# wwood/CoverM

Hardware: AMD Instinct MI355X
Metric: aligned reads/s through coverm contig (mean trimmed_mean covered_fraction variance) (higher is better)
Workload: dtype i32 depth / u64 sums / f32 estimators

## Files before the change

coverm_amd/csrc/covermhip.hip:

```cpp
#include "pileup_kernels.hip.h"
#include "prep_lean.hip.h"
#include "genome_kernels.hip.h"
#include "sep_kernels.hip.h"
#include "ingest_kernels.hip.h"
#include "group_kernels.hip.h"
#include "sam_kernels.hip.h"

#include <algorithm>
#include <atomic>
#include <cstddef>
#include <chrono>
#include <cstdio>
#include <dlfcn.h>
#include <functional>
#include <sched.h>
#include <cstdlib>
#include <cstring>
#include <map>
#include <mutex>
#include <string>
#include <future>
#include <thread>
#include <vector>

#include "../../include/covermhip.h"
#include "roctx_ranges.h"
#include "knobs.h"
#include "record_store.h"
#include "store_plan_core.h"

using namespace covk;

static_assert(sizeof(cov_config) == 40 && offsetof(cov_config, min_aligned_length) == 12 && offsetof(cov_config, min_percent_identity) == 16 &&
              offsetof(cov_config, contig_end_exclusion) == 24 && offsetof(cov_config, want) == 32, "cov_config layout");
static_assert(sizeof(cov_batch) == 80 && offsetof(cov_batch, cigar) == 64 && offsetof(cov_batch, n_records) == 72, "cov_batch layout");
static_assert(sizeof(cov_contig_stats) == 128 && offsetof(cov_contig_stats, sum_identity_primary) == 40 && offsetof(cov_contig_stats, win_sum_d) == 56 &&
              offsetof(cov_contig_stats, first_record) == 88 && offsetof(cov_contig_stats, win_min_d) == 104 && offsetof(cov_contig_stats, hist_len) == 112 &&
              offsetof(cov_contig_stats, hist_off) == 120, "cov_contig_stats layout");
static_assert(sizeof(cov_summary) == 32 && offsetof(cov_summary, hist_total) == 24, "cov_summary layout");
static_assert(sizeof(cov_interval) == 24 && sizeof(cov_interval_stats) == 56, "interval struct layout");
static_assert(sizeof(cov_genome_stats) == 24 && sizeof(cov_genome_stats) == sizeof(covk::DevGenomeStats) && offsetof(cov_genome_stats, genome_len) == offsetof(covk::DevGenomeStats, genome_len) &&
              offsetof(cov_genome_stats, any_nonzero) == offsetof(covk::DevGenomeStats, any_nonzero), "cov_genome_stats mirrors the device struct");
static_assert(sizeof(cov_genome_entry) == 24 && offsetof(cov_genome_entry, first_tid) == 8 && offsetof(cov_genome_entry, gid) == 12 && offsetof(cov_genome_entry, n_contigs_seen) == 16 &&
              offsetof(cov_genome_entry, any_nonzero) == 20 && sizeof(covk::SepEntry) == 8, "cov_genome_entry layout (numpy mirror in coverm_amd/native.py)");
static_assert(sizeof(cov_estimator) == sizeof(covk::DevEstimator) && offsetof(cov_estimator, contig_end_exclusion) == offsetof(covk::DevEstimator, excl) &&
              offsetof(cov_estimator, trim_max) == offsetof(covk::DevEstimator, trim_max) && COV_EST_MAX == covk::EST_MAX && COV_EST_ANIR == covk::EST_ANIR, "cov_estimator mirrors the device struct");

namespace {

#define HIPCHK(call)                                                                          \
    do {                                                                                      \
        hipError_t e_ = (call);                                                               \
        if (e_ != hipSuccess) {                                                               \
            char b_[512];                                                                     \
            snprintf(b_, sizeof b_, "%s failed: %s (%s:%d)", #call, hipGetErrorString(e_), __FILE__, __LINE__); \
            s->err = b_;                                                                      \
            return COV_ERR_HIP;                                                               \
        }                                                                                     \
    } while (0)

std::string g_create_error;

// ... 131 lines not shown
    uint64_t ing_first_record = 0;
    uint64_t ing_launched = 0;
    covi::BgzfBlock *h_blocks = nullptr; size_t h_blocks_cap = 0;
    uint64_t ing_comp = 0, ing_infl = 0, ing_blocks = 0;
    bool ing_active = false;
    InflateKernel ing_K;
    hipStream_t ing_copy = nullptr;
    std::future<hipError_t> ing_prep;
    hipEvent_t ing_ev[COV_INGEST_SLOTS] = {}, ing_fed = nullptr;
    double ing_s_alloc = 0;
    double ing_s_part[4] = {0, 0, 0, 0};

    bool sam_active = false, sam_seen_record = false, sam_decode_timed = false;
    uint64_t sam_window = 0, sam_expected = 0, sam_lines = 0, sam_bytes = 0, sam_err_line = 0;
    uint32_t sam_err = 0, sam_k = 0;
    DevBuf<uint8_t> m_text[2], m_blob;
    DevBuf<u64> m_nl, m_tab, m_res, m_noff;
    DevBuf<u32> m_line_end, m_cnt, m_rec_idx, m_cig_idx, m_bsum[3], m_slots;
    samc::Table m_names{};
    hipEvent_t sam_buf_free[2] = {}, sam_ev[4] = {};
    float sam_ms = 0.f; uint32_t sam_launches = 0;

    bool finished = false;
    uint8_t *h_res = nullptr; size_t h_res_cap = 0;
    std::future<std::pair<uint8_t *, size_t>> h_res_prep;
    DevContig *h_ctg = nullptr;
    DevGlobal h_glob{};
    bool last_gen_all = false;
    uint64_t algo_bytes = 0;

    hipEvent_t ev[COV_K_COUNT][2] = {};
    hipEvent_t ev_begin[COV_K_COUNT] = {};
    int ev_fresh = -1;
    float k_ms[COV_K_COUNT] = {};
    uint32_t k_launches[COV_K_COUNT] = {};
};

static cov_status spill_store(cov_session *s, bool &progress);

namespace {

size_t result_block_bytes(u32 n_targets) { return sizeof(DevGlobal) + (size_t)std::max<u32>(n_targets, 1) * sizeof(DevContig); }
static size_t result_host_bytes(const cov_session *s, u32 nT) {
    return result_block_bytes(nT) + (size_t)std::max<u32>(nT, 1) * ((s->have_mask || s->have_runs) ? 1u : std::max<u32>(s->est.n, 1u)) * sizeof(float);
}
static void result_host_take(cov_session *s) {
    if (!s->h_res_prep.valid()) return;
    const std::pair<uint8_t *, size_t> r = s->h_res_prep.get();
    if (!r.first) return;
    if (r.second > s->h_res_cap) {
        if (s->h_res) (void)hipHostFree(s->h_res);
        s->h_res = r.first; s->h_res_cap = r.second;
    } else (void)hipHostFree(r.first);
}

hipError_t bind_result_block(cov_session *s, u32 n_targets) {
    hipError_t e = s->d_res.reserve(result_block_bytes(n_targets) + (size_t)std::max<u32>(n_targets, 1) * COV_EST_MAX * sizeof(float), s->stream);
    if (e != hipSuccess) return e;
    s->d_glob.p = reinterpret_cast<DevGlobal *>(s->d_res.p); s->d_glob.cap = 1;
    s->d_ctg.p = reinterpret_cast<DevContig *>(s->d_res.p + sizeof(DevGlobal)); s->d_ctg.cap = std::max<u32>(n_targets, 1);
    return hipSuccess;
}

Records records_of(const cov_session *s) {
    Records r{};
    if (s->adopted) {
// ... 36 lines not shown
        const cov_status sp = spill_store(s, progress);
        if (sp != COV_OK) return sp;
        s->spill_retry_at = progress ? 0 : 2 * s->store.n_records;
    }
    if (s->store.n_records + n >= 0xfffffff0ull) { s->err = "more than 2^32 records of one reference (or of one batch) in the record store"; return COV_ERR_INVALID_ARG; }
    if (s->store.n_cigar + ncig >= 0xfffffff0ull) { s->err = "more than 2^32 CIGAR words of one reference (or of one batch) in the record store"; return COV_ERR_INVALID_ARG; }
    RecordStore &S = s->store;
    const uint64_t R = S.n_records, N = R + n; hipStream_t st = s->stream;
    HIPCHK(S.reserve(N, S.n_cigar + ncig + 1, st, R, S.n_cigar, false));
    HIPCHK(S.copy_in(*b, n, off0, ncig, kind, st));
    if (off0 != (u32)S.n_cigar) {
        const u32 cnt = (u32)(n + 1);
        hipLaunchKernelGGL(k_rebase_offsets, dim3((cnt + 255) / 256), dim3(256), 0, st, S.cigar_off.p + R, cnt, off0, (u32)S.n_cigar);
        HIPCHK(hipGetLastError());
    }
    S.n_records = N; S.n_cigar += ncig;
    s->finished = false;
    if (!from_device) HIPCHK(hipStreamSynchronize(st));
    return COV_OK;
}

cov_status materialise_adopted(cov_session *s) {
    if (!s->adopted) return COV_OK;
    const cov_batch ab = s->adopted_batch;
    s->adopted = false; s->store.n_records = 0; s->store.n_cigar = 0;
    return append(s, &ab, true);
}

void timing_events(cov_session *s) {
    if (s->ev[0][0]) return;
    for (int k = 0; k < COV_K_COUNT; k++)
        for (int j = 0; j < 2; j++) (void)hipEventCreate(&s->ev[k][j]);
}
void time_begin(cov_session *s, int k) {
    if (s->ev_fresh >= 0) { s->ev_begin[k] = s->ev[s->ev_fresh][1]; return; }
    (void)hipEventRecord(s->ev[k][0], s->stream); s->ev_begin[k] = s->ev[k][0];
}
void time_end(cov_session *s, int k) { (void)hipEventRecord(s->ev[k][1], s->stream); s->k_launches[k]++; s->ev_fresh = k; }

template <bool H, int TABLES>
void launch_fast_v(cov_session *s, const PileupArgs &a, u32 n_tiles) {
    const auto kern = TABLES == 1 ? &k_pileup_fast<H> : &k_pileup_fast2t<H>;
    const size_t smem = pileup_fast_smem_bytes(H, TABLES == 1 ? FAST_HB : FAST_HB7, TABLES);
    static std::atomic<int> occ_dev[64];
    std::atomic<int> &occ_slot = occ_dev[(unsigned)s->cfg.device & 63u];
    int occ = occ_slot.load(std::memory_order_relaxed);
    const u32 chunk = (u32)s->chunk_tiles;
    const u32 n_chunks = (n_tiles + chunk - 1) / chunk;
    if (!occ) {
        (void)hipFuncSetAttribute(reinterpret_cast<const void *>(kern), hipFuncAttributeMaxDynamicSharedMemorySize, (int)smem);
        int nb = 0;
        if (hipOccupancyMaxActiveBlocksPerMultiprocessor(&nb, reinterpret_cast<const void *>(kern), 256, smem) != hipSuccess || nb < 1) {
            (void)hipGetLastError();
            nb = (int)std::max<size_t>(1, std::min<size_t>(8, (160 * 1024) / smem));
        }
        occ = nb; occ_slot.store(nb, std::memory_order_relaxed);
    }
    const u32 wg_per_cu = 8u * (u32)occ;
    const u32 grid = std::max(1u, std::min((n_chunks + 3) / 4, (u32)s->n_cus * wg_per_cu));
    hipLaunchKernelGGL(kern, dim3(grid), dim3(256), smem, s->stream, a, n_tiles, chunk);
}
template <bool H>
void launch_fast_t(cov_session *s, const PileupArgs &a, u32 n_tiles) {
    if (s->fast_tables == 2) launch_fast_v<H, 2>(s, a, n_tiles);
    else launch_fast_v<H, 1>(s, a, n_tiles);
}

template <bool H, bool W>
void launch_stream_t(cov_session *s, const PileupArgs &a, u32 n_tiles, bool slow_list_only = false) {
    const size_t smem = pileup_stream_smem_bytes();
    static std::atomic<int> occ_dev[64];
    std::atomic<int> &occ_slot = occ_dev[(unsigned)s->cfg.device & 63u];
    int occ = occ_slot.load(std::memory_order_relaxed);
    const u32 chunk = (u32)s->chunk_tiles;
    const u32 n_chunks = (n_tiles + chunk - 1) / chunk;
    if (!occ) {
        (void)hipFuncSetAttribute(reinterpret_cast<const void *>(&k_pileup_stream<H, W>), hipFuncAttributeMaxDynamicSharedMemorySize, (int)smem);
        int nb = 0;
        if (hipOccupancyMaxActiveBlocksPerMultiprocessor(&nb, reinterpret_cast<const void *>(&k_pileup_stream<H, W>), 256, smem) != hipSuccess || nb < 1) {
            (void)hipGetLastError();
            nb = (int)std::max<size_t>(1, std::min<size_t>(8, (160 * 1024) / smem));
        }
        occ = nb; occ_slot.store(nb, std::memory_order_relaxed);
    }
    const u32 wg_per_cu = 8u * (u32)occ;
    if (slow_list_only) {
        hipLaunchKernelGGL((k_pileup_stream<H, W>), dim3((u32)s->n_cus), dim3(256), smem, s->stream, a, 0u, 1u,
                           (const u32 *)s->d_slow_list.p, (const u32 *)&s->d_glob.p->n_slow);
        return;
    }
    const u32 grid = std::max(1u, std::min((n_chunks + 3) / 4, (u32)s->n_cus * wg_per_cu));
    hipLaunchKernelGGL((k_pileup_stream<H, W>), dim3(grid), dim3(256), smem, s->stream, a, n_tiles, chunk, (const u32 *)nullptr,
                       (const u32 *)nullptr);
}
template <bool H, bool W>
void launch_any_pileup(cov_session *s, const PileupArgs &a, u32 n_tiles) {
    if (s->use_fast && !W) {
        launch_fast_t<H>(s, a, n_tiles);
        launch_stream_t<H, W>(s, a, n_tiles, true);
    } else launch_stream_t<H, W>(s, a, n_tiles);
}

PileupArgs pileup_args(cov_session *s) {
    PileupArgs a{};
    a.tile_contig = s->d_tile_contig.p; a.tile_start = s->d_tile_start.p; a.desc = s->d_desc.p;
    a.runs = s->d_runs.p; a.cx_runs = s->d_cx_runs.p; a.r = records_of(s); a.ctg = s->d_ctg.p; a.g = s->d_glob.p;
    a.hist_arena = s->d_arena.p; a.excl = s->cfg.contig_end_exclusion; a.depth_out = nullptr; a.tile_base = 0;
    return a;
}

}

extern "C" {

int cov_abi_version(void) { return COVERMHIP_ABI_VERSION; }

const char *cov_last_error(const cov_session *s) { return s ? s->err.c_str() : g_create_error.c_str(); }

static hipError_t ingest_prepare_(cov_session *s) {
    hipError_t e = hipSetDevice(s->cfg.device);
    if (e != hipSuccess || s->ing_copy) return e;
#define PREP(x) do { e = (x); if (e != hipSuccess) return e; } while (0)
    PREP(hipStreamCreateWithFlags(&s->ing_copy, hipStreamNonBlocking));
    for (int k = 0; k < COV_INGEST_SLOTS; k++) PREP(hipEventCreateWithFlags(&s->ing_ev[k], hipEventDisableTiming));
    PREP(hipEventCreateWithFlags(&s->ing_fed, hipEventDisableTiming));
    PREP(hipStreamCreateWithFlags(&s->ing_aux, hipStreamNonBlocking));
    PREP(hipStreamCreateWithFlags(&s->ing_parse, hipStreamNonBlocking));
    s->ing_ext = s->ing_parse;
    for (int k = 0; k < 2; k++) { PREP(hipEventCreateWithFlags(&s->ing_inf_done[k], hipEventDisableTiming)); PREP(hipEventCreateWithFlags(&s->ing_lz_done[k], hipEventDisableTiming)); }
    for (int k = 0; k < 4; k++) PREP(hipEventCreateWithFlags(&s->ing_ver_done[k], hipEventDisableTiming));
    for (int k = 0; k < 3; k++) { PREP(hipEventCreateWithFlags(&s->ing_ext_done[k], hipEventDisableTiming)); PREP(hipEventCreateWithFlags(&s->ing_cdone[k], hipEventDisableTiming)); }
// ... 20 lines not shown
    const bool timing = cov_timing_on();
    const auto tc0 = std::chrono::steady_clock::now();
    auto stamp = [&](const char *what) { if (timing) fprintf(stderr, "[covermhip] cov_create: %s at %.4fs\n", what, std::chrono::duration<double>(std::chrono::steady_clock::now() - tc0).count()); };
    int ndev = 0;
    hipError_t e = hipGetDeviceCount(&ndev);
    stamp("hipGetDeviceCount (runtime initialised)");
    if (e != hipSuccess || ndev <= 0) {
        g_create_error = std::string("no usable HIP device: ") + hipGetErrorString(e) +
                         " (the engine has no CPU fallback)";
        return COV_ERR_HIP;
    }
    if (cfg->device < 0 || cfg->device >= ndev) { g_create_error = "device ordinal out of range"; return COV_ERR_INVALID_ARG; }
    e = hipSetDevice(cfg->device);
    if (e != hipSuccess) { g_create_error = std::string("hipSetDevice: ") + hipGetErrorString(e); return COV_ERR_HIP; }
    cov_session *s = new cov_session();
    s->cfg = *cfg;
    {
        const char *mode = getenv("COVERM_PILEUP");
        if (mode && !strcmp(mode, "stream")) s->use_fast = false;
        s->tile = STREAM_TW;
        stamp("hipSetDevice");
        int cus = 0;
        if (hipDeviceGetAttribute(&cus, hipDeviceAttributeMultiprocessorCount, cfg->device) == hipSuccess && cus > 0) s->n_cus = cus;
        stamp("device attribute");
    }
    if (cfg->want & COV_WANT_INGEST) s->ing_prep = std::async(std::launch::async, [s] { return ingest_prepare_(s); });
    if (const char *el = getenv("COVERM_EST_LANES")) s->est_lanes = atoi(el) ? 1 : 0;
    if (const char *ft = getenv("COVERM_FAST_TABLES")) s->fast_tables = atoi(ft) == 2 ? 2 : 1;
    if (const char *pk = getenv("COVERM_PREP_KERNEL")) s->prep_kernel = atoi(pk) == 7 ? 7 : 0;
    if (const char *im = getenv("COVERM_IDENTITY")) s->id_mode = strcmp(im, "serial") ? 1 : 0;
    { long long v; if (covknob::get("store_cap_records", v) && v >= 1) s->cap_records = std::min<uint64_t>((uint64_t)v, 0xfffffff0ull); }
    { long long v; if (covknob::get("store_cap_cigar", v) && v >= 1) s->cap_cigar = std::min<uint64_t>((uint64_t)v, 0xfffffff0ull); }
    { long long v; if (covknob::get("pileup_chunk_tiles", v) && v >= 1 && v <= 64) s->chunk_tiles = (int)v; }
    e = hipEventCreateWithFlags(&s->ev_prep_done, hipEventDisableTiming);
    if (e == hipSuccess) e = hipEventCreateWithFlags(&s->ev_side_done, hipEventDisableTiming);
    if (e == hipSuccess) e = hipStreamCreateWithFlags(&s->stream, hipStreamNonBlocking);
    if (e != hipSuccess) { g_create_error = std::string("hipStreamCreate: ") + hipGetErrorString(e); (void)ingest_prep_wait(s); delete s; return COV_ERR_HIP; }
    stamp("streams and events");
    e = bind_result_block(s, 1);
    if (e != hipSuccess) { g_create_error = std::string("hipMalloc: ") + hipGetErrorString(e); cov_destroy(s); return COV_ERR_HIP; }
    stamp("first hipMalloc");
    *out = s;
    return COV_OK;
}

static void ingest_free_buffers(cov_session *s) {
    s->g_scratch.release(); s->g_carry.release(); s->g_blocks.release(); s->g_status.release();
    s->g_crc_tab.release();
    for (int k = 0; k < 3; k++) { s->g_win[k].release(); s->g_cwin[k].release(); }
    for (int k = 0; k < 4; k++) { s->g_seg[k].release(); s->g_recbase[k].release(); s->g_cigbase[k].release(); }
    s->g_tok.release(); s->g_ntok.release(); s->g_tok2.release(); s->g_ntok2.release();
    for (auto &b : s->m_text) b.release();
    s->m_nl.release(); s->m_tab.release(); s->m_line_end.release(); s->m_cnt.release(); s->m_rec_idx.release(); s->m_cig_idx.release();
}

void cov_destroy(cov_session *s) {
    if (!s) return;
    (void)ingest_prep_wait(s);
    (void)hipSetDevice(s->cfg.device);
    if (s->stream) (void)hipStreamSynchronize(s->stream);
    s->d_tlen.release(); s->d_tile_contig.release(); s->d_tile_start.release(); s->d_mask.release();
    s->d_grow.release(); s->d_gtids.release(); s->d_gseg_genome.release(); s->d_gseg_start.release(); s->d_genomes.release(); s->d_ghist.release(); s->d_ghist_top.release(); s->d_order.release();
    s->d_sgid.release(); s->d_sblk.release(); s->d_sent_pos.release(); s->d_stop_last1.release(); s->d_stop_first.release(); s->d_scounts.release(); s->d_scode.release();
    s->d_stop_cnt.release(); s->d_stop_seg.release(); s->d_sent.release();
    s->d_gout.release(); if (s->h_gout) (void)hipHostFree(s->h_gout); s->h_gout = nullptr;
    s->d_tile_first.release(); s->d_tcnt.release(); s->d_fov.release(); s->d_tscan.release(); s->d_ttop.release(); s->d_slow_list.release();
    s->d_ctg_scratch.release(); s->d_depth_all.release(); s->d_depth_off.release(); s->d_iv.release(); s->d_ivst.release(); s->d_ivhist.release();
    s->d_cx_list.release(); s->d_cx_cnt.release(); s->d_cx_cur.release(); s->d_cx_scan.release(); s->d_cx_top.release(); s->d_cx_runs.release();
    if (s->side) {
        (void)hipStreamSynchronize(s->side);
        if (s->side_owned) (void)hipStreamDestroy(s->side);
        s->side = nullptr; s->side_owned = false;
    }
    if (s->ing_aux) (void)hipStreamSynchronize(s->ing_aux);
    if (s->ing_parse) (void)hipStreamSynchronize(s->ing_parse);
    if (s->ing_ext) (void)hipStreamSynchronize(s->ing_ext);
    ingest_free_buffers(s);
    s->g_result.release();
    if (s->ing_aux) (void)hipStreamDestroy(s->ing_aux);
    if (s->ing_parse) (void)hipStreamDestroy(s->ing_parse);
    for (int k = 0; k < 2; k++) { if (s->ing_inf_done[k]) (void)hipEventDestroy(s->ing_inf_done[k]); if (s->ing_lz_done[k]) (void)hipEventDestroy(s->ing_lz_done[k]); }
    for (int k = 0; k < 4; k++) if (s->ing_ver_done[k]) (void)hipEventDestroy(s->ing_ver_done[k]);
    for (int k = 0; k < 3; k++) { if (s->ing_ext_done[k]) (void)hipEventDestroy(s->ing_ext_done[k]); if (s->ing_cdone[k]) (void)hipEventDestroy(s->ing_cdone[k]); }
    if (s->h_winres) (void)hipHostFree(s->h_winres);
    s->h_winres = nullptr;
    if (s->h_blocks) (void)hipHostFree(s->h_blocks);
    s->h_blocks = nullptr;
    if (s->ing_copy) { (void)hipStreamSynchronize(s->ing_copy); (void)hipStreamDestroy(s->ing_copy); }
    for (int k = 0; k < COV_INGEST_SLOTS; k++) if (s->ing_ev[k]) (void)hipEventDestroy(s->ing_ev[k]);
    for (hipEvent_t e : s->sam_buf_free) if (e) (void)hipEventDestroy(e);
    for (hipEvent_t e : s->sam_ev) if (e) (void)hipEventDestroy(e);
    for (auto &b : s->m_text) b.release();
    s->m_blob.release(); s->m_nl.release(); s->m_tab.release(); s->m_res.release(); s->m_noff.release(); s->m_line_end.release(); s->m_cnt.release();
    s->m_rec_idx.release(); s->m_cig_idx.release(); s->m_slots.release(); for (auto &b : s->m_bsum) b.release();
    if (s->ing_fed) (void)hipEventDestroy(s->ing_fed);
    s->d_res.release(); s->d_ctg.p = nullptr; s->d_glob.p = nullptr; s->d_desc.release(); s->d_gather.release();
    if (s->h_gather) (void)hipHostFree(s->h_gather);
    s->h_gather = nullptr;
    result_host_take(s);
    if (s->h_res) (void)hipHostFree(s->h_res);
    s->h_res = nullptr; s->h_res_cap = 0; s->h_ctg = nullptr;
    if (s->h_chist) (void)hipHostFree(s->h_chist);
    s->h_chist = nullptr; s->h_chist_cap = 0;
    s->h_estf = nullptr; s->store.release();
    s->d_runs.release(); s->d_part.release(); s->d_prep_args.release(); s->d_gen_list.release(); s->d_hist_top.release(); s->d_ident.release(); s->d_identp.release(); s->d_idch.release();
    if (s->ev_prep_done) (void)hipEventDestroy(s->ev_prep_done);
    if (s->ev_side_done) (void)hipEventDestroy(s->ev_side_done); s->d_arena.release(); s->d_chist.release(); s->d_depth.release();
    for (int k = 0; k < COV_K_COUNT; k++)
        for (int j = 0; j < 2; j++) if (s->ev[k][j]) (void)hipEventDestroy(s->ev[k][j]);
    if (s->stream) (void)hipStreamDestroy(s->stream);
    delete s;
}

static void genomes_off(cov_session *s) {
    if (s->have_genomes && (s->cfg.want & COV_WANT_IDENTITY_NONSUPP_ONLY))
        for (uint32_t k = 0; k < s->est.n; k++)
            if (s->est.e[k].kind == COV_EST_ANIR) { s->est = EstParams{}; s->est_valid = false; break; }
    s->have_genomes = false; s->have_runs = false; s->gen_valid = false;
}
cov_status cov_set_targets(cov_session *s, uint32_t n_targets, const uint64_t *target_len) {
    if (!s || (!target_len && n_targets)) return COV_ERR_INVALID_ARG;
    HIPCHK(hipSetDevice(s->cfg.device));
    s->n_targets = n_targets;
    s->h_tlen.resize(n_targets);
    s->h_tile_first.assign((size_t)n_targets + 1, 0);
    uint64_t nt = 0;
    for (uint32_t c = 0; c < n_targets; c++) {
        if (target_len[c] > 0x7fffffffull) { s->err = "target length exceeds BAM's i32 range"; return COV_ERR_INVALID_ARG; }
        s->h_tlen[c] = (uint32_t)target_len[c];
        s->h_tile_first[c] = (uint32_t)nt;
        nt += (target_len[c] + (uint64_t)s->tile - 1) / (uint64_t)s->tile;
    }
    if (nt >= 0x7fffffffull) { s->err = "too many tiles"; return COV_ERR_INVALID_ARG; }
    s->h_tile_first[n_targets] = (uint32_t)nt;
    s->n_tiles = (uint32_t)nt;
    std::vector<u32> tc(nt), ts(nt);
    for (uint32_t c = 0; c < n_targets; c++) {
        u32 k = s->h_tile_first[c];
        for (uint64_t p = 0; p < target_len[c]; p += (uint64_t)s->tile, k++) { tc[k] = c; ts[k] = (u32)p; }
    }
    HIPCHK(s->d_tlen.reserve(std::max<size_t>(1, n_targets), s->stream));
    HIPCHK(s->d_tile_contig.reserve(std::max<size_t>(1, nt), s->stream));
// ... 165 lines not shown
        return COV_OK;
    }
    { const cov_status st = materialise_adopted(s); if (st) return st; }
    return append(s, b, true);
}

cov_status cov_ingest_abort(cov_session *s) {
    if (!s) return COV_ERR_INVALID_ARG;
    if (!s->ing_active) return COV_OK;
    HIPCHK(hipSetDevice(s->cfg.device));
    s->ing_active = false; s->sam_active = false;
    for (hipStream_t st : {s->ing_copy, s->stream, s->ing_aux, s->ing_parse, s->ing_ext})
        if (st) HIPCHK(hipStreamSynchronize(st));
    s->ing_rec_total = s->ing_cig_total = 0; s->ing_round_n = 0; s->ing_fail = 0;
    s->ing_extracted = s->ing_batch;
    if (s->ing_rec_spilled) {
        s->ing_rec_spilled = 0;
        s->err = "cov_ingest_abort: part of the file had already left the bounded record store; cov_reset the session";
        return COV_ERR_STATE;
    }
    return COV_OK;
}

cov_status cov_reset(cov_session *s) {
    if (!s) return COV_ERR_INVALID_ARG;
    if (s->ing_active) {
        const bool spilled = s->ing_rec_spilled != 0;
        const cov_status a = cov_ingest_abort(s);
        if (a != COV_OK && !(spilled && a == COV_ERR_STATE)) return a;
        if (a != COV_OK) s->err.clear();
    }
    s->adopted = false; s->store.n_records = 0; s->store.n_cigar = 0; s->finished = false; s->depth_all_valid = false; s->store.mates_valid = 0; s->ing_was_span = false;
    s->spill.clear(); s->merged_valid = false; s->merged_hist.clear(); s->ing_rec_spilled = 0; s->spill_retry_at = 0; s->spill_est.clear(); s->est_valid = false; s->gen_valid = false;
    return COV_OK;
}

static cov_status convert_results(cov_session *s, const DevGlobal &G, const DevContig *ctg, uint64_t n_records, cov_contig_stats *stats,
                                  cov_summary *summary, int64_t min_ok_tid = -1, uint64_t rec_base = 0) {
    const u32 nT = s->n_targets;
    const bool want_hist = s->cfg.want & COV_WANT_HIST;
    if (G.internal_error) { s->err = "internal error: depth or histogram size exceeded its proven bound"; return COV_ERR_STATE; }
    uint64_t err_rec = ~0ull; int err_code = 0;
    if (G.first_error != ~0ull) { err_rec = G.first_error >> 8; err_code = (int)(G.first_error & 0xff); }
    const u32 n_chunks = nT >= 65536u ? std::min<u32>(8u, std::max<u32>(1u, std::thread::hardware_concurrency())) : 1u;
    const u32 per_chunk = (nT + n_chunks - 1) / std::max<u32>(n_chunks, 1u);
    auto chunked = [&](auto fn) {
        if (n_chunks <= 1) { fn(0u, 0u, nT); return; }
        std::vector<std::thread> th;
        for (u32 k = 1; k < n_chunks; k++) th.emplace_back([&, k] { fn(k, std::min(nT, k * per_chunk), std::min(nT, (k + 1) * per_chunk)); });
        fn(0u, 0u, std::min(nT, per_chunk));
        for (auto &t : th) t.join();
    };
    const bool want_hist_bins = want_hist;
    const u64 excl = s->cfg.contig_end_exclusion;
    std::vector<uint64_t> ch_last(n_chunks, 0), ch_bins(n_chunks, 0), ch_unsorted(n_chunks, ~0ull);
    std::vector<uint8_t> ch_any(n_chunks, 0);
    if (n_chunks > 1)
        chunked([&](u32 k, u32 lo, u32 hi) {
            uint64_t last = 0, bins = 0; bool any = false;
            for (u32 c = lo; c < hi; c++) {
                const DevContig &C = ctg[c];
                if (C.n_pass == 0) continue;
                last = any ? std::max<uint64_t>(last, C.last_rec) : C.last_rec; any = true;
                if (want_hist_bins) {
                    const u64 L = s->h_tlen[c];
                    if (2 * excl < L && (!s->have_mask || s->h_mask[c])) bins += C.max_d + 1u;
// ... 76 lines not shown
static cov_status verdict_results(cov_session *s, const DevGlobal &G, uint64_t unsorted_at, uint64_t n_records, cov_summary *summary) {
    if (G.internal_error) { s->err = "internal error: depth or histogram size exceeded its proven bound"; return COV_ERR_STATE; }
    uint64_t err_rec = ~0ull; int err_code = 0;
    if (G.first_error != ~0ull) { err_rec = G.first_error >> 8; err_code = (int)(G.first_error & 0xff); }
    if (unsorted_at != ~0ull && unsorted_at <= err_rec) {
        s->err = "BAM file appears to be unsorted. Input BAM files must be sorted by reference (i.e. by samtools sort)";
        return COV_ERR_UNSORTED;
    }
    if (err_code) {
        char b[256];
        const char *what = err_code == 2 ? "Mapping record encountered that does not have an 'NM' auxiliary tag in the SAM/BAM format"
                         : err_code == 3 ? "Unexpected data type of NM aux tag"
                         : err_code == 4 ? "aligned block starts at or beyond the end of its reference sequence"
                         : err_code == 7 ? "record refers to a reference id outside the header (Corrupt BAM file?)"
                                         : "invalid CIGAR operation";
        snprintf(b, sizeof b, "%s (record %llu)", what, (unsigned long long)err_rec);
        s->err = b;
        return (cov_status)err_code;
    }
    if (summary) {
        uint64_t prim = 0, cons = 0;
        for (u32 k = 0; k < COUNTER_SLOTS * 8; k++) { prim += G.prim_slots[k]; cons += G.cons_slots[k]; }
        summary->num_detected_primary_alignments = prim; summary->n_records = n_records; summary->n_considered = cons; summary->hist_total = 0;
    }
    return COV_OK;
}

static cov_status finish_once(cov_session *s, cov_contig_stats *stats, cov_summary *summary, bool &again);

static cov_status finish_store(cov_session *s, cov_contig_stats *stats, cov_summary *summary) {
    bool again = false;
    cov_status st = finish_once(s, stats, summary, again);
    if (st == COV_OK && again) st = finish_once(s, stats, summary, again);
    if (st == COV_OK && again) { s->err = "internal error: bucket sizing did not converge"; return COV_ERR_STATE; }
    return st;
}

static cov_status merge_spilled(cov_session *s, cov_contig_stats *stats, cov_summary *summary);

cov_status cov_finish(cov_session *s, cov_contig_stats *stats, cov_summary *summary) {
    covr::Range rr("cov_finish");
    if (s) s->merged_valid = false;
    cov_summary local;
    cov_status st = finish_store(s, stats, (s && s->spill.active && !summary) ? &local : summary);
    if (st == COV_OK && s->spill.active) st = merge_spilled(s, stats, summary ? summary : &local);
    return st;
}

cov_status cov_finish_genomes(cov_session *s, cov_summary *summary) {
    covr::Range rr("cov_finish_genomes");
    if (!s) return COV_ERR_INVALID_ARG;
    s->merged_valid = false;
    if (s->spill.active) { s->err = "cov_finish_genomes: part of the sample's contigs left the bounded record store: cov_finish, and aggregate on the host"; return COV_ERR_STATE; }
    s->lean_finish = true;
    const cov_status st = finish_store(s, nullptr, summary);
    s->lean_finish = false;
    return st;
}

static cov_status finish_once(cov_session *s, cov_contig_stats *stats, cov_summary *summary, bool &again) {
    again = false;
    if (!s || (!stats && s->n_targets && !s->lean_finish)) return COV_ERR_INVALID_ARG;
    const bool lean = s->lean_finish;
    s->depth_all_valid = false;
    HIPCHK(hipSetDevice(s->cfg.device));
    timing_events(s);
// ... 12 lines not shown
    const uint64_t ncig_all = s->adopted ? s->adopted_ncig : s->store.n_cigar;
    const bool long_cigars = R && ncig_all / R >= 16;
    const int prep_kernel = s->prep_kernel;
    const int prep_passes = long_cigars ? 1 : 2 * PREP_PASSES, prep_b = 1;
    const u32 prep_chunk = (u32)(256 * prep_b * prep_passes);
    const u32 prep_grid = (R + prep_chunk - 1) / prep_chunk;
    HIPCHK(s->d_part.reserve((size_t)prep_grid + 2, st));
    if (want_id) {
        if (!(s->cfg.want & COV_WANT_IDENTITY_PRIMARY_ONLY)) HIPCHK(s->d_ident.reserve(std::max<size_t>(1, R), st));
        if (!(s->cfg.want & COV_WANT_IDENTITY_NONSUPP_ONLY)) HIPCHK(s->d_identp.reserve(std::max<size_t>(1, R), st));
        HIPCHK(s->d_idch.reserve((size_t)R / ID_CH + 2, st));
    }
    if (want_hist) HIPCHK(s->d_arena.reserve((size_t)R + nT + 1, st));

    TileIdx ti{};
    ti.tile_first = s->d_tile_first.p; ti.tcnt = s->d_tcnt.p; ti.fov = s->d_fov.p; ti.shift = s->tile_shift; ti.n_tiles = s->n_tiles;
    CxIdx cx{};
    {
        const uint64_t ncig_now = s->adopted ? s->adopted_ncig : s->store.n_cigar;
        HIPCHK(s->d_cx_list.reserve((size_t)(ncig_now / CX_MIN_OPS) + 64, st));
        cx.list = s->d_cx_list.p; cx.list_cap = (u32)std::min<uint64_t>(ncig_now / CX_MIN_OPS + 64, 0xffffffffull);
        cx.cnt = s->d_cx_cnt.p; cx.cur = s->d_cx_cur.p; cx.cscan = s->d_cx_scan.p; cx.ctop = s->d_cx_top.p;
        cx.runs = s->d_cx_runs.p; cx.runs_cap = s->d_cx_runs.cap;
    }
    const Records r = records_of(s);
    const uint8_t *mask = s->have_mask ? s->d_mask.p : nullptr;
    FilterCfg f{};
    f.include_improper_pairs = s->cfg.include_improper_pairs; f.include_supplementary = s->cfg.include_supplementary;
    f.include_secondary = s->cfg.include_secondary; f.filter_single = s->cfg.filter_single;
    f.min_mapq = s->cfg.min_mapq; f.min_aligned_length = s->cfg.min_aligned_length;
    f.min_percent_identity = s->cfg.min_percent_identity; f.min_aligned_percent = s->cfg.min_aligned_percent;
    double *idp = (want_id && !(s->cfg.want & COV_WANT_IDENTITY_NONSUPP_ONLY)) ? s->d_identp.p : nullptr;
    double *idn = (want_id && !(s->cfg.want & COV_WANT_IDENTITY_PRIMARY_ONLY)) ? s->d_ident.p : nullptr;
    HIPCHK(s->d_prep_args.reserve(1, st));
    HIPCHK(s->d_gen_list.reserve((size_t)R / 64 + 2, st));
    PrepArgs pa{};
    {
        PrepHot &ph = pa.hot;
        ph.tid = r.tid; ph.pos = r.pos; ph.flag = r.flag; ph.nmk = r.nm_kind; ph.nm = r.nm; ph.coff = r.cigar_off; ph.cigar = r.cigar; ph.mapq = r.mapq; ph.lseq = r.l_seq;
        ph.runs = s->d_runs.p; ph.tcnt = ti.tcnt; ph.fov = ti.fov; ph.identp = idp; ph.identn = idn;
        ph.n = r.n; ph.cigar_end = r.cigar_end; ph.n_targets = nT; ph.shift = ti.shift; ph.steps = (u32)prep_chunk / 256u;
        ph.gate_mask = 0x4u | (f.include_secondary ? 0u : 0x100u) | (f.include_supplementary ? 0u : 0x800u) | (f.include_improper_pairs ? 0u : 0x2u);
        ph.p1_mask = 0x4u | (f.include_secondary ? 0u : 0x100u) | (f.include_supplementary ? 0u : 0x800u);
        ph.min_mapq = f.min_mapq; ph.min_aligned_length = f.min_aligned_length; ph.min_percent_identity = f.min_percent_identity; ph.min_aligned_percent = f.min_aligned_percent;
        PrepCold &pc = pa.cold;
        pc.ctg = s->d_ctg.p; pc.g = s->d_glob.p; pc.part = s->d_part.p; pc.cx_list = cx.list; pc.mask = mask; pc.tlen = s->d_tlen.p; pc.tile_first = s->d_tile_first.p;
        pc.cx_list_cap = cx.list_cap; pc.gen_list = s->d_gen_list.p;
    }
    hipLaunchKernelGGL(k_init, dim3((std::max(std::max(nT, COUNTER_SLOTS * 8), s->n_tiles) + 255) / 256), dim3(256), 0, st, s->d_ctg.p,
                       nT, s->d_glob.p, ti, cx, s->d_prep_args.p, pa);
    HIPCHK(hipGetLastError());

    if (R) {
        time_begin(s, COV_K_PREP);
        const u32 n_steps = (R + 63u) / 64u;
        const bool gen_all = prep_kernel != 7 && (uint64_t)R < (uint64_t)nT * 128u;
        s->last_gen_all = gen_all;
        const u32 gen_grid = gen_all ? std::min<u32>((u32)s->n_cus * 64u, (n_steps + 3u) / 4u) : std::min<u32>((u32)s->n_cus * 8u, (n_steps + 3u) / 4u);
#define COV_LAUNCH_PREP(ID, FI, MA)                                                                                                       \
        do {                                                                                                                              \
            if (prep_kernel == 7)                                                                                                         \
                hipLaunchKernelGGL((k_prep7s<ID, FI, MA>), dim3(prep_grid), dim3(256), 0, st, r, s->d_tlen.p, nT, mask, f, s->d_ctg.p,   \
                                   s->d_glob.p, s->d_runs.p, idp, idn, s->d_part.p, ti, prep_passes, prep_b, cx.list, cx.list_cap);      \
            else if (gen_all)                                                                                                             \
                hipLaunchKernelGGL((k_prep_generic<ID, FI, MA>), dim3(gen_grid), dim3(256), 0, st, (const PrepArgs *)s->d_prep_args.p, n_steps); \
            else {                                                                                                                        \
                hipLaunchKernelGGL((k_prep_lean<ID, FI, MA>), dim3(prep_grid), dim3(256), 0, st, pa.hot, (const PrepArgs *)s->d_prep_args.p); \
                hipLaunchKernelGGL((k_prep_generic<ID, FI, MA>), dim3(gen_grid), dim3(256), 0, st, (const PrepArgs *)s->d_prep_args.p, 0u); \
            }                                                                                                                             \
        } while (0)
        {
            const int key = (want_id ? 4 : 0) | (s->cfg.filter_single ? 2 : 0) | (mask != nullptr ? 1 : 0);
            switch (key) {
            case 0: COV_LAUNCH_PREP(false, false, false); break;
            case 1: COV_LAUNCH_PREP(false, false, true); break;
            case 2: COV_LAUNCH_PREP(false, true, false); break;
            case 3: COV_LAUNCH_PREP(false, true, true); break;
            case 4: COV_LAUNCH_PREP(true, false, false); break;
            case 5: COV_LAUNCH_PREP(true, false, true); break;
            case 6: COV_LAUNCH_PREP(true, true, false); break;
            default: COV_LAUNCH_PREP(true, true, true); break;
            }
        }
#undef COV_LAUNCH_PREP
        if (nT) {
            const u32 n_red = gen_all ? 0u : (nT + 3u) / 4u, cx_grid0 = (u32)s->n_cus * 8u;
            hipLaunchKernelGGL(k_post_prep, dim3(n_red + cx_grid0), dim3(256), 0, st, r, s->d_tlen.p, s->d_glob.p, cx, ti, s->d_ctg.p, nT, (const PrepPartial *)s->d_part.p,
                               prep_grid, prep_chunk, n_red);
        }
        time_end(s, COV_K_PREP);
        HIPCHK(hipGetLastError());
        if (want_id && nT) {
            if (!s->side) {
                (void)ingest_prep_wait(s);
                if (s->ing_aux && !s->ing_active) s->side = s->ing_aux;
                else { HIPCHK(hipStreamCreateWithFlags(&s->side, hipStreamNonBlocking)); s->side_owned = true; }
            }
            HIPCHK(hipEventRecord(s->ev_prep_done, st));
            HIPCHK(hipStreamWaitEvent(s->side, s->ev_prep_done, 0));
            (void)hipEventRecord(s->ev[COV_K_IDENTITY][0], s->side);
            if (s->id_mode) {
                const u32 nch = (R + ID_CH - 1) / ID_CH;
                hipLaunchKernelGGL(k_id_approx, dim3(nch), dim3(256), 0, s->side, idp, idn, R, s->d_idch.p);
                hipLaunchKernelGGL(k_id_predict, dim3(nT), dim3(64), 0, s->side, s->d_ctg.p, nT, idp, idn, s->d_idch.p);
                hipLaunchKernelGGL(k_id_exact, dim3(nch), dim3(256), 0, s->side, idp, idn, R, s->d_idch.p);
                hipLaunchKernelGGL(k_id_combine, dim3(nT), dim3(64), 0, s->side, s->d_ctg.p, nT, idp, idn, r.tid, s->d_idch.p);
            } else
                hipLaunchKernelGGL(k_identity, dim3(nT), dim3(64), 0, s->side, s->d_ctg.p, nT, idp, idn, r.tid);
            (void)hipEventRecord(s->ev[COV_K_IDENTITY][1], s->side);
            s->k_launches[COV_K_IDENTITY]++;
            HIPCHK(hipGetLastError());
            HIPCHK(hipEventRecord(s->ev_side_done, s->side));
            s->ev_fresh = -1;
        }
    }
    if (R && s->n_tiles) {
        time_begin(s, COV_K_RANGES);
        const u32 n_blocks = (s->n_tiles + 1023u) / 1024u;
        const u32 cx_grid = (u32)s->n_cus * 8u;
        ScanPair sp{};
        sp.cnt[0] = s->d_tcnt.p; sp.scan[0] = s->d_tscan.p; sp.top[0] = s->d_ttop.p; sp.total[0] = nullptr;
        sp.cnt[1] = s->d_cx_cnt.p; sp.scan[1] = s->d_cx_scan.p; sp.top[1] = s->d_cx_top.p; sp.total[1] = &s->d_glob.p->cx_total;
        hipLaunchKernelGGL(k_tile_scan1, dim3(2u * n_blocks), dim3(1024), 0, st, sp, s->n_tiles, n_blocks);
        hipLaunchKernelGGL(k_tile_scan2, dim3(2), dim3(1024), 0, st, sp, n_blocks);
        hipLaunchKernelGGL((k_cx_expand<true>), dim3(cx_grid), dim3(256), 0, st, r, s->d_tlen.p, s->d_glob.p, cx, ti);
        u32 *slow_list = s->use_fast ? s->d_slow_list.p : nullptr;
        if (want_hist)
            hipLaunchKernelGGL((k_ranges<true>), dim3((s->n_tiles + 255) / 256), dim3(256), 0, st, s->d_tile_contig.p,
                               s->d_tile_start.p, s->n_tiles, s->d_tlen.p, mask, s->d_ctg.p, s->d_desc.p, ti, s->d_tscan.p,
                               s->d_ttop.p, cx, s->d_glob.p, slow_list);
        else
            hipLaunchKernelGGL((k_ranges<false>), dim3((s->n_tiles + 255) / 256), dim3(256), 0, st, s->d_tile_contig.p,
                               s->d_tile_start.p, s->n_tiles, s->d_tlen.p, mask, s->d_ctg.p, s->d_desc.p, ti, s->d_tscan.p,
                               s->d_ttop.p, cx, s->d_glob.p, slow_list);
        time_end(s, COV_K_RANGES);
        HIPCHK(hipGetLastError());
        if (want_hist) {
            time_begin(s, COV_K_HIST);
            const u32 hb = (nT + 1023u) / 1024u;
            HIPCHK(s->d_hist_top.reserve(hb, st));
            hipLaunchKernelGGL((k_hist_sum<0>), dim3(hb), dim3(1024), 0, st, (const DevContig *)s->d_ctg.p, nT, s->d_tlen.p, mask, (u64)s->cfg.contig_end_exclusion, s->d_hist_top.p);
            hipLaunchKernelGGL((k_hist_off<0>), dim3(hb), dim3(1024), 0, st, s->d_ctg.p, nT, s->d_tlen.p, mask, (u64)s->cfg.contig_end_exclusion, (const u64 *)s->d_hist_top.p, s->d_glob.p);
            hipLaunchKernelGGL(k_zero_u32, dim3(2048), dim3(256), 0, st, s->d_arena.p, &s->d_glob.p->hist_cap_total);
            time_end(s, COV_K_HIST);
            HIPCHK(hipGetLastError());
        }
        PileupArgs a = pileup_args(s);
        compacted = want_hist && (s->est.n == 0 || s->hist_fetch_seen);
        derive_in_est = want_hist && !compacted && !(s->have_mask || s->have_runs) && s->est.n != 0;
        time_begin(s, COV_K_PILEUP);
        if (want_hist) launch_any_pileup<true, false>(s, a, s->n_tiles);
        else launch_any_pileup<false, false>(s, a, s->n_tiles);
        if (want_hist && !derive_in_est) {
            if (est_lanes) hipLaunchKernelGGL((k_hist_stats<true>), dim3((nT + 255) / 256), dim3(256), 0, st, s->d_ctg.p, nT, (const u32 *)s->d_tlen.p, mask, (u64)s->cfg.contig_end_exclusion, (const u32 *)s->d_arena.p);
            else hipLaunchKernelGGL((k_hist_stats<false>), dim3((nT + 3) / 4), dim3(256), 0, st, s->d_ctg.p, nT, (const u32 *)s->d_tlen.p, mask, (u64)s->cfg.contig_end_exclusion, (const u32 *)s->d_arena.p);
        }
        time_end(s, COV_K_PILEUP);
        HIPCHK(hipGetLastError());
        if (want_hist) {
            s->hist_prefetched = 0;
            if (compacted) {
                HIPCHK(s->d_chist.reserve((size_t)R + nT + 1, st));
                time_begin(s, COV_K_HIST_COMPACT);
                const u32 hb = (nT + 1023u) / 1024u;
                hipLaunchKernelGGL((k_hist_sum<1>), dim3(hb), dim3(1024), 0, st, (const DevContig *)s->d_ctg.p, nT, s->d_tlen.p, mask, (u64)s->cfg.contig_end_exclusion, s->d_hist_top.p);
                hipLaunchKernelGGL((k_hist_off<1>), dim3(hb), dim3(1024), 0, st, s->d_ctg.p, nT, s->d_tlen.p, mask, (u64)s->cfg.contig_end_exclusion, (const u64 *)s->d_hist_top.p, s->d_glob.p);
                hipLaunchKernelGGL(k_hist_compact, dim3((nT + 3u) / 4u), dim3(256), 0, st, s->d_ctg.p, nT, s->d_tlen.p, (u64)s->cfg.contig_end_exclusion, s->d_arena.p, s->d_chist.p);
                time_end(s, COV_K_HIST_COMPACT);
                HIPCHK(hipGetLastError());
                const u64 guess = s->hist_fetch_seen ? std::min<u64>({s->last_chist_total + s->last_chist_total / 16, (u64)R + nT + 1, (u64)(64u << 20) / 8}) : 0;
                if (guess) {
                    if (guess > s->h_chist_cap) {
                        if (s->h_chist) (void)hipHostFree(s->h_chist);
                        s->h_chist = nullptr; s->h_chist_cap = 0;
                        HIPCHK(hipHostMalloc((void **)&s->h_chist, (size_t)guess * 8, hipHostMallocDefault));
                        s->h_chist_cap = guess;
                    }
                    HIPCHK(hipMemcpyAsync(s->h_chist, s->d_chist.p, (size_t)guess * 8, hipMemcpyDeviceToHost, st));
                    s->hist_prefetched = guess;
                }
            }
            s->hist_fetch_seen = false;
        }
    }
    const size_t block = result_block_bytes(nT), nf = (s->have_mask || s->have_runs) ? 0 : (size_t)nT * s->est.n;
    {
        result_host_take(s);
        const size_t need = lean ? sizeof(DevGlobal) + sizeof(DevContig) : result_host_bytes(s, nT);
        if (need > s->h_res_cap) {
            if (s->h_res) (void)hipHostFree(s->h_res);
            s->h_res = nullptr; s->h_res_cap = 0;
            const size_t cap = need < ((size_t)64 << 20) ? need + need / 2 : need;
            HIPCHK(hipHostMalloc((void **)&s->h_res, cap, hipHostMallocDefault));
            s->h_res_cap = cap;
        }
        s->h_ctg = (DevContig *)(s->h_res + sizeof(DevGlobal));
        s->h_estf = reinterpret_cast<float *>(s->h_res + block);
    }
    if (want_id && R && nT) { HIPCHK(hipStreamWaitEvent(st, s->ev_side_done, 0)); s->ev_fresh = -1; }
// ... 66 lines not shown
        if (runs) HIPCHK(hipMemcpyAsync(s->h_gout + (size_t)nG * (sizeof(DevGenomeStats) + s->est.n * sizeof(float)), s->d_sent.p, (size_t)nG * sizeof(SepEntry), hipMemcpyDeviceToHost, st));
    }
    if (lean) {
        const u32 ob = (nT + 1023u) / 1024u;
        HIPCHK(s->d_order.reserve((size_t)ob + 2, st));
        hipLaunchKernelGGL(k_order_max, dim3(std::max(ob, 1u)), dim3(1024), 0, st, (const DevContig *)s->d_ctg.p, nT, s->d_order.p);
        hipLaunchKernelGGL(k_order_check, dim3(std::max(ob, 1u)), dim3(1024), 0, st, (const DevContig *)s->d_ctg.p, nT, s->d_order.p);
        HIPCHK(hipGetLastError());
        HIPCHK(hipMemcpyAsync(s->h_res, s->d_res.p, sizeof(DevGlobal), hipMemcpyDeviceToHost, st));
        HIPCHK(hipMemcpyAsync(s->h_res + sizeof(DevGlobal), s->d_order.p, 8, hipMemcpyDeviceToHost, st));
    } else
    HIPCHK(hipMemcpyAsync(s->h_res, s->d_res.p, sizeof(DevGlobal) + (size_t)nT * sizeof(DevContig) + (nf ? (block - sizeof(DevGlobal) - (size_t)nT * sizeof(DevContig)) + nf * sizeof(float) : 0),
                          hipMemcpyDeviceToHost, st));
    {
        const auto t_spin = std::chrono::steady_clock::now();
        for (;;) {
            const hipError_t q = hipStreamQuery(st);
            if (q == hipSuccess) break;
            if (q != hipErrorNotReady) { (void)hipGetLastError(); break; }
            (void)hipGetLastError();
            if (std::chrono::steady_clock::now() - t_spin > std::chrono::milliseconds(4)) break;
            __builtin_ia32_pause();
        }
    }
    HIPCHK(hipStreamSynchronize(st));
    memcpy(&s->h_glob, s->h_res, sizeof(DevGlobal));
    if (s->h_glob.cx_total > s->d_cx_runs.cap) {
        const uint64_t need = s->h_glob.cx_total + s->h_glob.cx_total / 8 + 1024;
        s->d_cx_runs.release();
        HIPCHK(s->d_cx_runs.reserve((size_t)need, st));
        again = true;
        return COV_OK;
    }
    for (int k = 0; k < COV_K_COUNT; k++)
        if (s->k_launches[k]) (void)hipEventElapsedTime(&s->k_ms[k], k == COV_K_IDENTITY ? s->ev[k][0] : s->ev_begin[k], s->ev[k][1]);

    {
        const uint64_t ncig = s->adopted ? s->adopted_ncig : s->store.n_cigar;
        s->algo_bytes = (uint64_t)R * 24 + ncig * 4 + (uint64_t)nT * sizeof(DevContig);
    }

    if (lean) {
        u64 unsorted_at; memcpy(&unsorted_at, s->h_res + sizeof(DevGlobal), 8);
        const cov_status cst = verdict_results(s, s->h_glob, unsorted_at, R, summary);
        if (cst != COV_OK) return cst;
        s->last_chist_total = 0; s->hist_compacted = false; s->est_valid = false; s->gen_valid = true; s->finished = true;
        return COV_OK;
    }
    const cov_status cst = convert_results(s, s->h_glob, s->h_ctg, R, stats, summary, s->spill.inflight, s->spill.records);
    if (cst != COV_OK) return cst;
    s->last_chist_total = 0;
    if (want_hist) for (u32 c = 0; c < nT; c++) s->last_chist_total += stats[c].hist_len;
    s->hist_compacted = compacted;
    s->est_valid = s->est.n != 0 && !s->have_mask && !s->have_runs;
    s->gen_valid = genomes;
    s->finished = true;
    return COV_OK;
}


static cov_status fetch_chunk_hist(cov_session *s, uint64_t *hist);

static cov_status spill_store(cov_session *s, bool &progress) {
    progress = false;
    if (s->adopted || s->store.n_records == 0 || s->want_mates || s->n_targets == 0) return COV_OK;
    covr::Range rr("bounded store: spill");
    const u32 nT = s->n_targets;
    const bool want_hist = s->cfg.want & COV_WANT_HIST;
// ... 1072 lines not shown
cov_status cov_ingest_copy_inflated(cov_session *s, uint64_t offset, uint64_t n, void *out) {
    if (!s || offset + n > s->ing_infl || (n && !out)) return COV_ERR_INVALID_ARG;
    if (s->ing_batch != 1) { s->err = "cov_ingest_copy_inflated: the file was parsed in several windows, the stream is gone"; return COV_ERR_STATE; }
    HIPCHK(hipSetDevice(s->cfg.device));
    HIPCHK(hipMemcpyAsync(out, s->g_win[0].p + inflate_kernel(s).carry + offset, n, hipMemcpyDeviceToHost, s->stream));
    HIPCHK(hipStreamSynchronize(s->stream));
    return COV_OK;
}

cov_status cov_fetch_hist(cov_session *s, uint64_t *hist) {
    if (!s || !s->finished || !(s->cfg.want & COV_WANT_HIST)) return COV_ERR_STATE;
    if (s->merged_valid) {
        s->hist_fetch_seen = true;
        if (s->merged_hist.empty()) return COV_OK;
        if (!hist) return COV_ERR_INVALID_ARG;
        memcpy(hist, s->merged_hist.data(), s->merged_hist.size() * 8);
        return COV_OK;
    }
    return fetch_chunk_hist(s, hist);
}

static cov_status fetch_chunk_hist(cov_session *s, uint64_t *hist) {
    if (!s || !s->finished || !(s->cfg.want & COV_WANT_HIST)) return COV_ERR_STATE;
    HIPCHK(hipSetDevice(s->cfg.device));
    const uint64_t total = s->last_chist_total;
    s->hist_fetch_seen = true;
    if (total == 0) return COV_OK;
    if (!hist) return COV_ERR_INVALID_ARG;
    if (!s->hist_compacted) {
        HIPCHK(s->d_chist.reserve(total, s->stream));
        const uint8_t *mask = s->have_mask ? (const uint8_t *)s->d_mask.p : (const uint8_t *)nullptr;
        const u32 hb = (s->n_targets + 1023u) / 1024u;
        HIPCHK(s->d_hist_top.reserve(hb, s->stream));
        hipLaunchKernelGGL((k_hist_sum<1>), dim3(hb), dim3(1024), 0, s->stream, (const DevContig *)s->d_ctg.p, s->n_targets, s->d_tlen.p, mask, (u64)s->cfg.contig_end_exclusion, s->d_hist_top.p);
        hipLaunchKernelGGL((k_hist_off<1>), dim3(hb), dim3(1024), 0, s->stream, s->d_ctg.p, s->n_targets, s->d_tlen.p, mask, (u64)s->cfg.contig_end_exclusion, (const u64 *)s->d_hist_top.p, s->d_glob.p);
        hipLaunchKernelGGL(k_hist_compact, dim3((s->n_targets + 3u) / 4u), dim3(256), 0, s->stream, s->d_ctg.p, s->n_targets, s->d_tlen.p,
                           (u64)s->cfg.contig_end_exclusion, s->d_arena.p, s->d_chist.p);
        HIPCHK(hipGetLastError());
        s->hist_prefetched = 0; s->hist_compacted = true;
    }
    const u64 have = std::min<u64>(total, s->hist_prefetched);
    if (have) memcpy(hist, s->h_chist, (size_t)have * 8);
    if (have < total) {
        HIPCHK(hipMemcpyAsync(hist + have, s->d_chist.p + have, (size_t)(total - have) * 8, hipMemcpyDeviceToHost, s->stream));
        HIPCHK(hipStreamSynchronize(s->stream));
    }
    return COV_OK;
}

cov_status cov_copy_depth(cov_session *s, uint32_t tid, int32_t *depth_out) {
    if (!s || !s->finished) return COV_ERR_STATE;
    if (s->spill.active) { s->err = "cov_copy_depth: part of the sample's records already left the bounded record store"; return COV_ERR_STATE; }
    if (tid >= s->n_targets || !depth_out) return COV_ERR_INVALID_ARG;
    HIPCHK(hipSetDevice(s->cfg.device));
    const u32 L = s->h_tlen[tid];
    if (L == 0) return COV_OK;
    HIPCHK(s->d_depth.reserve(L, s->stream));
    HIPCHK(hipMemsetAsync(s->d_depth.p, 0, (size_t)L * 4, s->stream));
    PileupArgs a = pileup_args(s);
    DevBuf<DevContig> &scratch = s->d_ctg_scratch;
    HIPCHK(scratch.reserve(s->n_targets, s->stream));
    HIPCHK(hipMemcpyAsync(scratch.p, s->d_ctg.p, (size_t)s->n_targets * sizeof(DevContig), hipMemcpyDeviceToDevice, s->stream));
    a.ctg = scratch.p;
    a.depth_out = s->d_depth.p;
    a.tile_base = s->h_tile_first[tid];
    const u32 grid = s->h_tile_first[tid + 1] - s->h_tile_first[tid];
    launch_any_pileup<false, true>(s, a, grid);
    HIPCHK(hipGetLastError());
// ... 61 lines not shown
    if (hist_total) *hist_total = s->ivhist_total;
    return COV_OK;
}

cov_status cov_fetch_interval_hist(cov_session *s, uint64_t *hist) {
    if (!s || !s->finished) return COV_ERR_STATE;
    if (s->ivhist_total == 0) return COV_OK;
    if (!hist) return COV_ERR_INVALID_ARG;
    HIPCHK(hipSetDevice(s->cfg.device));
    HIPCHK(hipMemcpyAsync(hist, s->d_ivhist.p, s->ivhist_total * 8, hipMemcpyDeviceToHost, s->stream));
    HIPCHK(hipStreamSynchronize(s->stream));
    return COV_OK;
}

cov_status cov_kernel_ms(const cov_session *s, cov_kernel_id k, double *ms_total, uint32_t *launches) {
    if (!s || k < 0 || k >= COV_K_COUNT) return COV_ERR_INVALID_ARG;
    if (k == COV_K_SAM) {
        if (ms_total) *ms_total = s->sam_ms;
        if (launches) *launches = s->sam_launches;
        return COV_OK;
    }
    if (k == COV_K_GROUP) {
        if (ms_total) *ms_total = s->grp_ms[0];
        if (launches) *launches = s->grp_launches;
        return COV_OK;
    }
    if (ms_total) *ms_total = s->k_ms[k];
    if (launches) *launches = s->k_launches[k];
    return COV_OK;
}

cov_status cov_last_paths(const cov_session *s, cov_path_counts *out) {
    if (!s || !out) return COV_ERR_INVALID_ARG;
    out->listed_steps = s->h_glob.n_gen; out->generic_only = s->last_gen_all ? 1u : 0u;
    out->slow_tiles = s->h_glob.n_slow; out->bucket_records = s->h_glob.n_cx;
    return COV_OK;
}

uint32_t cov_store_spills(const cov_session *s) { return s ? s->spill.count : 0u; }

cov_status cov_set_estimators(cov_session *s, const cov_estimator *est, uint32_t n_est) {
    if (!s || (n_est && !est)) return COV_ERR_INVALID_ARG;
    if (n_est > COV_EST_MAX) { s->err = "cov_set_estimators: more than COV_EST_MAX estimators"; return COV_ERR_INVALID_ARG; }
    if (s->spill.active) { s->err = "cov_set_estimators: set them before the sample's first records (part of it already left the bounded record store)"; return COV_ERR_STATE; }
    for (uint32_t k = 0; k < n_est; k++) {
        const int kind = est[k].kind;
        if (kind < 0 || kind > COV_EST_ANIR || kind == COV_EST_TPM || kind == COV_EST_PILEUP_COUNTS) {
            s->err = "cov_set_estimators: this estimator is evaluated on the host (TPM: f64 exp / ln of the host's libm; coverage histogram: prints the histogram itself)";
            return COV_ERR_INVALID_ARG;
        }
        if (kind == COV_EST_TRIMMED_MEAN && !(s->cfg.want & COV_WANT_HIST)) { s->err = "cov_set_estimators: a trimmed mean needs COV_WANT_HIST"; return COV_ERR_INVALID_ARG; }
        if (kind == COV_EST_ANIR && s->have_genomes) {
            if (!(s->cfg.want & COV_WANT_IDENTITY) || (s->cfg.want & COV_WANT_IDENTITY_PRIMARY_ONLY)) {
                s->err = "cov_set_estimators: ANIr of a genome needs COV_WANT_IDENTITY with the not-supplementary sum"; return COV_ERR_INVALID_ARG;
            }
        } else if (kind == COV_EST_ANIR && (!(s->cfg.want & COV_WANT_IDENTITY) || (s->cfg.want & COV_WANT_IDENTITY_NONSUPP_ONLY))) {
            s->err = "cov_set_estimators: ANIr needs COV_WANT_IDENTITY with the primary-read sum"; return COV_ERR_INVALID_ARG;
        }
    }
    s->est = EstParams{};
    for (uint32_t k = 0; k < n_est; k++) memcpy(&s->est.e[k], &est[k], sizeof(cov_estimator));
    s->est.n = n_est;
    s->est_valid = false; s->gen_valid = false;
    return COV_OK;
}

static cov_status genome_fetch_ready(cov_session *s, const char *what) {
    if (!s) return COV_ERR_INVALID_ARG;
// ... 159 lines not shown
```

coverm_amd/csrc/pileup_kernels.hip.h:

```cpp
#pragma once
#include <hip/hip_runtime.h>
#include <stdint.h>

#define HSTC_FN __host__ __device__ __forceinline__
#include "hist_stats_core.h"

namespace covk {

typedef unsigned long long u64;
typedef unsigned int u32;

constexpr u32 F_POS_UNSORTED = 1u;
constexpr u32 RW_SINGLE = 0u, RW_DOUBLE = 1u, RW_COMPLEX = 2u, RW_BUCKET = 3u;
constexpr u32 FAST_MAX_CAND = 8191u;
constexpr u32 TILE_F_GENERIC = 1u, TILE_F_SLOW = 2u;
constexpr u32 CX_MIN_OPS = 16;

struct DevContig {
    u64 n_primary, n_pass, n_nonsupp, sum_nm, sum_indel;
    double id_primary, id_nonsupp;
    u64 sum_d, sum_d2, cov_win, cov_full, proc_win;
    u64 hist_off;
    u32 first_rec, last_rec;
    u32 rec_start, rec_end;
    u32 n_groups;
    u32 max_span;
    u32 flags;
    u32 hist_cap;
    u32 min_d, max_d;
    u32 hist_len;
    u32 cov_out;
    u64 chist_off;
};
static_assert(sizeof(DevContig) == 160, "DevContig layout");

constexpr u32 COUNTER_SLOTS = 64;
struct DevGlobal {
    u64 first_error;
    u64 hist_cap_total;
    u64 chist_total;
    u32 internal_error;
    u32 n_cx;
    u64 cx_total;
    u32 n_slow;
    u32 n_gen;
    u64 pad2[2];
    u64 prim_slots[COUNTER_SLOTS * 8];
    u64 cons_slots[COUNTER_SLOTS * 8];
    u32 pad_q[8 * 16];
};

struct FilterCfg {
    u32 include_improper_pairs, include_supplementary, include_secondary;
    u32 filter_single, min_mapq, min_aligned_length;
    float min_percent_identity, min_aligned_percent;
};

struct Records {
    const int32_t *tid, *pos;
    const uint16_t *flag;
    const uint8_t *mapq;
    const u32 *nm;
    const uint8_t *nm_kind;
    const u32 *l_seq;
    const u32 *cigar_off;
    const u32 *cigar;
    u32 n;
    u32 cigar_end;
};

__device__ __forceinline__ int lane_id() { return threadIdx.x & 63; }

__device__ __forceinline__ int wave_incl_scan(int v) {
    v += __builtin_amdgcn_update_dpp(0, v, 0x111, 0xf, 0xf, false);
    v += __builtin_amdgcn_update_dpp(0, v, 0x112, 0xf, 0xf, false);
    v += __builtin_amdgcn_update_dpp(0, v, 0x114, 0xf, 0xf, false);
    v += __builtin_amdgcn_update_dpp(0, v, 0x118, 0xf, 0xf, false);
    v += __builtin_amdgcn_update_dpp(0, v, 0x142, 0xa, 0xf, false);
    v += __builtin_amdgcn_update_dpp(0, v, 0x143, 0xc, 0xf, false);
    return v;
}
__device__ __forceinline__ int wave_incl_max(int v) {
    const int NEG = (int)0x80000000;
// ... 39 lines not shown
__device__ __forceinline__ double bcast_f64(double v, int q) {
    const long long b = __double_as_longlong(v);
    const u32 lo = __builtin_amdgcn_readlane((u32)b, q), hi = __builtin_amdgcn_readlane((u32)(b >> 32), q);
    return __longlong_as_double((long long)(((u64)hi << 32) | lo));
}
__device__ __forceinline__ u64 bcast_u64(u64 v, int q) {
    const u32 lo = __builtin_amdgcn_readlane((u32)v, q), hi = __builtin_amdgcn_readlane((u32)(v >> 32), q);
    return ((u64)hi << 32) | lo;
}

__device__ __forceinline__ void report_error(DevGlobal *g, u32 rec, u32 code) {
    atomicMin(&g->first_error, ((u64)rec << 8) | code);
}

struct TileIdx {
    const u32 *tile_first;
    u32 *tcnt, *fov;
    u32 shift;
    u32 n_tiles;
};

struct CxIdx {
    u32 *list; u32 list_cap;
    u32 *cnt, *cur;
    const u32 *cscan, *ctop;
    uint2 *runs; u64 runs_cap;
};

struct PrepPartial;
struct PrepCold {
    DevContig *ctg; DevGlobal *g; PrepPartial *part; u32 *cx_list;
    const uint8_t *mask; const u32 *tlen; const u32 *tile_first;
    u32 *gen_list;
    u32 cx_list_cap, pad;
};
struct PrepHot {
    const int32_t *tid, *pos;
    const uint16_t *flag;
    const uint8_t *nmk;
    const u32 *nm, *coff, *cigar;
    const uint8_t *mapq;
    const u32 *lseq;
    uint2 *runs;
    u32 *tcnt, *fov;
    double *identp, *identn;
    u32 n, cigar_end, n_targets, shift, steps;
    u32 gate_mask;
    u32 p1_mask;
    u32 min_mapq, min_aligned_length;
    float min_percent_identity, min_aligned_percent;
};
struct PrepArgs { PrepHot hot; PrepCold cold; };

__global__ void k_init(DevContig *ctg, u32 n_targets, DevGlobal *g, TileIdx ti, CxIdx cx, PrepArgs *pa_out, PrepArgs pa) {
    u32 c = blockIdx.x * blockDim.x + threadIdx.x;
    if (c == 0 && pa_out != nullptr) *pa_out = pa;
    if (c < ti.n_tiles) { ti.tcnt[c] = 0u; ti.fov[c] = 0xffffffffu; cx.cnt[c] = 0u; cx.cur[c] = 0u; }
    if (c == 0) {
        g->first_error = ~0ull; g->hist_cap_total = 0; g->chist_total = 0; g->internal_error = 0;
        g->n_cx = 0; g->cx_total = 0; g->n_slow = 0; g->n_gen = 0;
    }
    if (c < COUNTER_SLOTS * 8) { g->prim_slots[c] = 0; g->cons_slots[c] = 0; }
    if (c >= n_targets) return;
    DevContig z;
    z.n_primary = z.n_pass = z.n_nonsupp = z.sum_nm = z.sum_indel = 0;
    z.id_primary = z.id_nonsupp = 0.0;
    z.sum_d = z.sum_d2 = z.cov_win = z.cov_full = z.proc_win = 0;
    z.hist_off = 0;
    z.first_rec = 0xffffffffu; z.last_rec = 0;
    z.rec_start = 0xffffffffu; z.rec_end = 0;
    z.n_groups = 0; z.max_span = 0; z.flags = 0; z.hist_cap = 0;
    z.min_d = 0xffffffffu; z.max_d = 0; z.hist_len = 0; z.cov_out = 0; z.chist_off = 0;
    ctg[c] = z;
}

constexpr int PREP_B = 2;
constexpr int PREP_PASSES = 8;
constexpr int PREP_CHUNK = 256 * PREP_B * PREP_PASSES;

constexpr u32 CIG_FAST_OPS = 128;
__device__ __forceinline__ void cigar_walk_slow(const u32 *__restrict__ cigar, u32 co0, u32 nops, int pos, u32 L, u64 &aligned,
                                             u64 &indel, u32 &run_start, u32 &run_len, u32 &run2_start, u32 &run2_len,
                                             u32 &n_runs, u32 &span, bool &oob, bool &badcig) {
    aligned = 0; indel = 0; run_start = run_len = run2_start = run2_len = n_runs = span = 0; oob = false; badcig = false;
    long long cursor = pos;
    long long cur_e = -1;
    for (u32 c = 0; c < nops; c++) {
        const u32 wd = cigar[co0 + c];
        const u32 op = wd & 15u, len = wd >> 4;
// ... 425 lines not shown
                o.tid = t0;
                for (int k = 0; k < 4; k++) {
                    const PrepPartial &q = wpart[k];
                    if (q.tid < 0) continue;
                    o.prim += q.prim; o.pass += q.pass; o.nons += q.nons; o.span = max(o.span, q.span);
                    o.first = min(o.first, q.first); o.last = max(o.last, q.last); o.nm += q.nm; o.indel += q.indel;
                }
            }
            part[blockIdx.x] = o;
        }
    }
    if (!uniform_wg) prep_flush(ctg, cur, acc);
    if (threadIdx.x == 0) {
        const u32 p = blk_cnt[0][0] + blk_cnt[0][1] + blk_cnt[0][2] + blk_cnt[0][3];
        const u32 c = blk_cnt[1][0] + blk_cnt[1][1] + blk_cnt[1][2] + blk_cnt[1][3];
        const u32 slot = (blockIdx.x % COUNTER_SLOTS) * 8u;
        if (p) atomicAdd(&g->prim_slots[slot], (u64)p);
        if (c) atomicAdd(&g->cons_slots[slot], (u64)c);
    }
}

#define COV_PREP_KERNEL(NAME, ATTR, PF, PB)                                                                                                           \
    template <bool WANT_IDENTITY, bool FILTER, bool MASKED>                                                                                      \
    __global__ __launch_bounds__(256) ATTR void NAME(Records r, const u32 *__restrict__ tlen, u32 n_targets, const uint8_t *__restrict__ mask,   \
                                                     FilterCfg f, DevContig *ctg, DevGlobal *g, uint2 *__restrict__ runs,                        \
                                                     double *__restrict__ identp, double *__restrict__ identn, PrepPartial *__restrict__ part,   \
                                                     TileIdx ti, int passes, int b_active, u32 *__restrict__ cx_list, u32 cx_list_cap) {         \
        prep_body<WANT_IDENTITY, FILTER, MASKED, PF, PB>(r, tlen, n_targets, mask, f, ctg, g, runs, identp, identn, part, ti, passes, b_active, cx_list, \
                                                 cx_list_cap);                                                                                   \
    }
COV_PREP_KERNEL(k_prep7s, __attribute__((amdgpu_waves_per_eu(7, 7))), true, 1)
#undef COV_PREP_KERNEL

__device__ __forceinline__ void prep_reduce_body(u32 c, DevContig *ctg, u32 n_targets, const PrepPartial *__restrict__ part, u32 n_parts, u32 chunk_recs) {
    if (c >= n_targets) return;
    DevContig *C = &ctg[c];
    const u32 rs = C->rec_start, re = C->rec_end;
    if (rs >= re) return;
    const u32 b0 = rs / chunk_recs, b1 = min((re - 1) / chunk_recs, n_parts - 1);
    u32 prim = 0, pass = 0, nons = 0, span = 0, first = 0xffffffffu, last = 0;
    u64 nm = 0, indel = 0;
    for (u32 b = b0 + (threadIdx.x & 63); b <= b1; b += 64) {
        const PrepPartial q = part[b];
        if (q.tid != (int)c) continue;
        prim += q.prim; pass += q.pass; nons += q.nons; span = max(span, q.span);
        first = min(first, q.first); last = max(last, q.last); nm += q.nm; indel += q.indel;
    }
    prim = wave_sum_u32(prim); pass = wave_sum_u32(pass); nons = wave_sum_u32(nons); span = wave_max_u32(span);
    first = wave_min_u32(first); last = wave_max_u32(last); nm = wave_sum_u64(nm); indel = wave_sum_u64(indel);
    if ((threadIdx.x & 63) == 0 && pass) {
        C->n_primary += prim; C->n_pass += pass; C->n_nonsupp += nons; C->sum_nm += nm; C->sum_indel += indel;
        C->max_span = max(C->max_span, span); C->first_rec = min(C->first_rec, first); C->last_rec = max(C->last_rec, last);
    }
}

__device__ __forceinline__ u32 lower_bound_pos(const int32_t *__restrict__ pos, u32 lo, u32 hi, long long key) {
    while (lo < hi) {
        const u32 mid = lo + ((hi - lo) >> 1);
        if ((long long)pos[mid] < key) lo = mid + 1; else hi = mid;
    }
    return lo;
}

struct ScanPair { const u32 *cnt[2]; u32 *scan[2]; u32 *top[2]; u64 *total[2]; };
__global__ __launch_bounds__(1024) void k_tile_scan1(ScanPair sp, u32 n_tiles, u32 n_blocks) {
    __shared__ u32 wtot[16];
    const u32 which = blockIdx.x >= n_blocks ? 1u : 0u, blk = blockIdx.x - which * n_blocks;
    const u32 *__restrict__ tcnt = sp.cnt[which];
// ... 4 lines not shown
    if (lane == 63) wtot[w] = inc;
    __syncthreads();
    u32 wbase = 0, tot = 0;
    for (int k = 0; k < 16; k++) { const u32 x = wtot[k]; if (k < w) wbase += x; tot += x; }
    if (t < n_tiles) sp.scan[which][t] = wbase + inc - v;
    if (threadIdx.x == 0) sp.top[which][blk] = tot;
}

__global__ __launch_bounds__(1024) void k_tile_scan2(ScanPair sp, u32 n_blocks) {
    __shared__ u32 wtot[16];
    __shared__ u32 carry_s;
    u32 *ttop = sp.top[blockIdx.x];
    u64 *total = sp.total[blockIdx.x];
    if (threadIdx.x == 0) carry_s = 0;
    __syncthreads();
    const int lane = lane_id(), w = threadIdx.x >> 6;
    for (u32 base = 0; base < n_blocks; base += 1024u) {
        const u32 b = base + threadIdx.x;
        const u32 v = b < n_blocks ? ttop[b] : 0u;
        const u32 inc = (u32)wave_incl_scan((int)v);
        if (lane == 63) wtot[w] = inc;
        __syncthreads();
        u32 wbase = 0, tot = 0;
        for (int k = 0; k < 16; k++) { const u32 x = wtot[k]; if (k < w) wbase += x; tot += x; }
        const u32 carry = carry_s;
        if (b < n_blocks) ttop[b] = carry + wbase + inc - v;
        __syncthreads();
        if (threadIdx.x == 0) carry_s = carry + tot;
        __syncthreads();
    }
    if (total != nullptr && threadIdx.x == 0) *total = carry_s;
}

template <bool FILL>
__device__ __forceinline__ void cx_expand_body(const Records &r, const u32 *__restrict__ tlen, DevGlobal *g, const CxIdx &cx, const TileIdx &ti, u32 wave, u32 n_waves) {
    const int lane = lane_id();
    const u32 n = min(g->n_cx, cx.list_cap);
    if (FILL && g->cx_total > cx.runs_cap) return;
    const u64 lt = lane == 0 ? 0ull : (~0ull >> (64 - lane));
    for (u32 j = wave; j < n; j += n_waves) {
        const u32 i = cx.list[j];
        const int tid = r.tid[i];
        const u32 co0 = r.cigar_off[i], nops = r.cigar_off[i + 1] - co0;
        const u32 L = tlen[tid], t0 = ti.tile_first[tid];
        long long cur0 = r.pos[i];
        u32 wd_next = (u32)lane < nops ? r.cigar[co0 + (u32)lane] : 4u;
        for (u32 base = 0; base < nops; base += 64) {
            const u32 wd = wd_next;
            const u32 idn = base + 64u + (u32)lane;
            wd_next = idn < nops ? r.cigar[co0 + idn] : 4u;
            const u32 len = wd >> 4, bit = 1u << (wd & 15u);
            const u32 fr = (bit & 0x18du) ? len : 0u;
            const u32 incl = (u32)wave_incl_scan((int)fr), excl = incl - fr;
            const long long sj = cur0 + (long long)excl;
            const bool m = (bit & 0x181u) != 0u && len > 0u && sj >= 0 && sj < (long long)L;
            const u32 sv = (u32)sj, ev = sv + len;
            const u32 ts = sv >> ti.shift, te = m ? (min(ev, L) - 1u) >> ti.shift : 0u;
            for (u32 k = 0; __any(m && ts + k <= te); k++) {
                const bool v = m && ts + k <= te;
                const u32 key = t0 + ts + k;
                u32 slot = 0;
                for (u64 todo = __ballot(v); todo != 0;) {
                    const int l = __ffsll((long long)todo) - 1;
                    const u32 k0 = __builtin_amdgcn_readlane(key, l);
                    const u64 grp = __ballot(v && key == k0);
                    u32 b = 0;
                    if (lane == l) b = atomicAdd(FILL ? &cx.cur[k0] : &cx.cnt[k0], (u32)__popcll(grp));
                    if (FILL) {
                        b = __builtin_amdgcn_readlane(b, l);
                        if (v && key == k0) slot = b + (u32)__popcll(grp & lt);
                    }
                    todo &= ~grp;
                }
                if (FILL && v) cx.runs[(u64)cx.cscan[key] + cx.ctop[key >> 10] + slot] = make_uint2(sv, ev);
            }
            cur0 += (long long)__builtin_amdgcn_readlane(incl, 63);
        }
    }
}

template <bool FILL>
__global__ __launch_bounds__(256) void k_cx_expand(Records r, const u32 *__restrict__ tlen, DevGlobal *g, CxIdx cx, TileIdx ti) {
    cx_expand_body<FILL>(r, tlen, g, cx, ti, blockIdx.x * 4u + (threadIdx.x >> 6), gridDim.x * 4u);
}

__global__ __launch_bounds__(256) void k_post_prep(Records r, const u32 *__restrict__ tlen, DevGlobal *g, CxIdx cx, TileIdx ti, DevContig *ctg, u32 n_targets,
                                                   const PrepPartial *__restrict__ part, u32 n_parts, u32 chunk_recs, u32 n_red) {
    if (blockIdx.x < n_red) prep_reduce_body(blockIdx.x * 4u + (threadIdx.x >> 6), ctg, n_targets, part, n_parts, chunk_recs);
    else cx_expand_body<false>(r, tlen, g, cx, ti, (blockIdx.x - n_red) * 4u + (threadIdx.x >> 6), (gridDim.x - n_red) * 4u);
}

template <bool WANT_HIST>
__global__ __launch_bounds__(256) void k_ranges(const u32 *__restrict__ tile_contig, const u32 *__restrict__ tile_start,
                                                u32 n_tiles, const u32 *__restrict__ tlen, const uint8_t *__restrict__ mask,
                                                DevContig *ctg, uint4 *__restrict__ desc, TileIdx ti,
                                                const u32 *__restrict__ tscan, const u32 *__restrict__ ttop, CxIdx cx,
                                                DevGlobal *__restrict__ g, u32 *__restrict__ slow_list) {
    const u32 t = blockIdx.x * blockDim.x + threadIdx.x;
    if (t >= n_tiles) return;
    const u32 c = tile_contig[t];
    DevContig *C = &ctg[c];
    uint4 out = make_uint4(0u, 0u, tlen[c], 0u);
    u32 cxn = 0, cxo = 0;
    if (C->n_pass != 0 && (mask == nullptr || mask[c])) {
        const u32 rs = C->rec_start, re = C->rec_end;
        cxn = g->cx_total <= cx.runs_cap ? cx.cnt[t] : 0u;
        cxo = cx.cscan[t] + cx.ctop[t >> 10];
        if (C->n_groups != 1u) out.w = 1u;
        if (C->n_groups != 1u || (C->flags & F_POS_UNSORTED)) {
            out.x = rs; out.y = re;
        } else {
            const u32 tf = ti.tile_first[c];
            const u32 before = (tscan[t] + ttop[t >> 10]) - (tscan[tf] + ttop[tf >> 10]);
            const u32 f = rs + before;
            out.y = min(f + ti.tcnt[t], re);
            out.x = max(min(f, ti.fov[t]), rs);
            out.x = min(out.x, out.y);
        }
    }
    if (out.x < out.y || cxn) {
        if (out.w || out.y - out.x + cxn > FAST_MAX_CAND) {
            out.w |= TILE_F_SLOW;
            if (slow_list != nullptr) slow_list[atomicAdd(&g->n_slow, 1u)] = t;
        }
    }
    if (WANT_HIST) {
        const u32 npass = (u32)min(C->n_pass, (u64)0xffffffffu);
        const u32 cap = min(out.y - out.x + cxn, npass);
        if (__all(c == (u32)__builtin_amdgcn_readfirstlane((int)c))) {
            const u32 m = wave_max_u32(cap);
            if (lane_id() == 0 && m) atomicMax(&C->hist_cap, m);
        } else if (cap) atomicMax(&C->hist_cap, cap);
    }
    desc[2 * t] = out;
    desc[2 * t + 1] = make_uint4(c, tile_start[t], cxo, cxn);
}

template <int MODE>
__device__ __forceinline__ u64 hist_bins_of(const DevContig *C, u32 c, const u32 *__restrict__ tlen, const uint8_t *__restrict__ mask, u64 excl) {
    const bool live = C->n_pass != 0 && (mask == nullptr || mask[c]);
    if (MODE == 0) return live ? (u64)C->hist_cap + 1 : 0;
    return (live && 2 * excl < (u64)tlen[c]) ? (u64)C->max_d + 1 : 0;
}
__device__ __forceinline__ u64 block_incl_scan_u64(u64 v, u64 *wtot, u64 &total) {
    const int lane = lane_id(), w = threadIdx.x >> 6;
    u64 inc = v;
#pragma unroll
    for (int o = 1; o < 64; o <<= 1) {
        const u64 t = __shfl_up(inc, o);
        if (lane >= o) inc += t;
    }
    if (lane == 63) wtot[w] = inc;
    __syncthreads();
    u64 wbase = 0; total = 0;
    for (int k = 0; k < 16; k++) { const u64 x = wtot[k]; if (k < w) wbase += x; total += x; }
    __syncthreads();
    return wbase + inc;
}
template <int MODE>
__global__ __launch_bounds__(1024) void k_hist_sum(const DevContig *__restrict__ ctg, u32 n_targets, const u32 *__restrict__ tlen,
                                                   const uint8_t *__restrict__ mask, u64 excl, u64 *__restrict__ top) {
    __shared__ u64 wtot[16];
    const u32 c = blockIdx.x * 1024u + threadIdx.x;
    u64 total;
    (void)block_incl_scan_u64(c < n_targets ? hist_bins_of<MODE>(&ctg[c], c, tlen, mask, excl) : 0, wtot, total);
    if (threadIdx.x == 0) top[blockIdx.x] = total;
}
template <int MODE>
__global__ __launch_bounds__(1024) void k_hist_off(DevContig *ctg, u32 n_targets, const u32 *__restrict__ tlen, const uint8_t *__restrict__ mask,
                                                   u64 excl, const u64 *__restrict__ top, DevGlobal *g) {
    __shared__ u64 wtot[16];
    u64 mine = 0, base;
    for (u32 b = threadIdx.x; b < blockIdx.x; b += 1024u) mine += top[b];
    (void)block_incl_scan_u64(mine, wtot, base);
    const u32 c = blockIdx.x * 1024u + threadIdx.x;
    const u64 v = c < n_targets ? hist_bins_of<MODE>(&ctg[c], c, tlen, mask, excl) : 0;
    u64 total;
    const u64 inc = block_incl_scan_u64(v, wtot, total);
    if (c < n_targets) {
        if (MODE == 0) ctg[c].hist_off = base + inc - v;
        else { ctg[c].chist_off = base + inc - v; ctg[c].hist_len = (u32)v; }
    }
    if (blockIdx.x == gridDim.x - 1 && threadIdx.x == 0) {
        if (MODE == 0) g->hist_cap_total = base + total; else g->chist_total = base + total;
    }
}

__global__ void k_zero_u32(u32 *__restrict__ p, const u64 *__restrict__ n_ptr) {
    const u64 n = *n_ptr;
    for (u64 i = (u64)blockIdx.x * blockDim.x + threadIdx.x; i < n; i += (u64)gridDim.x * blockDim.x) p[i] = 0u;
}

__global__ __launch_bounds__(256) void k_hist_compact(const DevContig *__restrict__ ctg, u32 n_targets,
                                                      const u32 *__restrict__ tlen, u64 excl,
                                                      const u32 *__restrict__ arena, u64 *__restrict__ out) {
    const u32 c = blockIdx.x * 4u + (threadIdx.x >> 6);
    if (c >= n_targets) return;
    const DevContig *C = &ctg[c];
    const u32 n = C->hist_len;
    if (n == 0) return;
    const u64 win_len = (u64)tlen[c] - 2 * excl;
    for (u32 d = threadIdx.x & 63u; d < n; d += 64u) {
        u64 v = arena[C->hist_off + d];
        if (d == 0) v += win_len - C->proc_win;
        out[C->chist_off + d] = v;
    }
}

__global__ __launch_bounds__(64) void k_identity(DevContig *ctg, u32 n_targets, const double *__restrict__ identp,
                                                 const double *__restrict__ identn, const int32_t *__restrict__ tidv) {
    const u32 c = blockIdx.x;
    if (c >= n_targets) return;
    DevContig *C = &ctg[c];
    if (C->n_pass == 0) return;
    const u32 rs = C->rec_start, re = C->rec_end;
    const bool generic = C->n_groups != 1u;
    double accp = 0.0, accn = 0.0;
    const int lane = lane_id();
    u32 i = rs + (u32)lane;
    double xp = 0.0, xn = 0.0;
    if (i < re && (!generic || tidv[i] == (int)c)) { if (identp) xp = identp[i]; if (identn) xn = identn[i]; }
    for (u32 b = rs; b < re; b += 64) {
        const double cp = xp, cn = xn;
// ... 225 lines not shown
                        const u64 T = bcast_u64(P, (int)(jstar - 1));
                        S = __longlong_as_double((long long)((bits & 0xfff0000000000000ull) | ((m + T) & 0xfffffffffffffull)));
                    }
                    if (jstar < nb) serial((kb + jstar) * ID_CH, (kb + jstar + 1) * ID_CH, is_p, !is_p);
                    q = jstar + 1;
                }
            };
            if (identp != nullptr) run_stream(Sp, x.ep, x.tp, (x.flags & (1u | 4u)) != 0u, true);
            if (identn != nullptr) run_stream(Sn, x.en, x.tn, (x.flags & (2u | 8u)) != 0u, false);
        }
        serial(k1 * ID_CH, re, true, true);
    }
    if (lane == 0) { C->id_primary = Sp; C->id_nonsupp = Sn; }
}

__device__ __attribute__((noinline)) void hist_add_overflow(u32 *arena, u64 hoff, u32 hcap, DevGlobal *g, u32 d, u32 x) {
    if (d <= hcap) atomicAdd(&arena[hoff + d], x);
    else atomicOr(&g->internal_error, 1u);
}

struct PileupArgs {
    const u32 *tile_contig, *tile_start;
    const uint4 *desc;
    const uint2 *runs;
    const uint2 *cx_runs;
    Records r;
    DevContig *ctg;
    DevGlobal *g;
    u32 *hist_arena;
    u64 excl;
    int32_t *depth_out;
    const u64 *depth_off;
    u32 tile_base;
};


__device__ __forceinline__ void lds_fence() { asm volatile("s_waitcnt lgkmcnt(0)" ::: "memory"); }

constexpr int STREAM_TW = 1024, STREAM_HB = 512, STREAM_CAP = 512;

template <bool WANT_HIST, bool WRITE_DEPTH>
__global__ __launch_bounds__(256) void k_pileup_stream(PileupArgs a, u32 n_tiles, u32 chunk_tiles,
                                                       const u32 *__restrict__ tile_list, const u32 *__restrict__ n_list) {
    if (tile_list != nullptr) n_tiles = *n_list;
    constexpr int TW = STREAM_TW, HBW = STREAM_HB, CAP = STREAM_CAP, ROWS = TW / 64;
    extern __shared__ __attribute__((aligned(16))) char smem[];
    const int lane = threadIdx.x & 63, w = threadIdx.x >> 6;
    int *tile = reinterpret_cast<int *>(smem + (size_t)w * (TW * 4 + HBW * 4));
    u32 *lhist = reinterpret_cast<u32 *>(tile + TW);
    int4 *t4 = reinterpret_cast<int4 *>(tile);
    int2 *ent = reinterpret_cast<int2 *>(tile);
    const u32 wave_id = blockIdx.x * 4u + (u32)w, n_waves = gridDim.x * 4u;
    if (WANT_HIST) {
#pragma unroll
        for (int b = lane; b < HBW; b += 64) lhist[b] = 0u;
    }
    u64 sum_d = 0, sum_d2 = 0, proc_win = 0;
    u32 cov_w = 0, cov_f = 0, mn = 0xffffffffu, mx = 0;
    u32 cov_o = 0;
    u32 hbound = 0;
    int cur_c = -1;
    u64 hoff = 0; u32 hcap = 0;
    const u64 excl = a.excl;

    auto hist_add = [&](u32 d, u32 x) {
        if (__builtin_expect(d < (u32)HBW, 1)) atomicAdd(&lhist[d], x);
// ... 256 lines not shown
                if (__any(cov_o != 0u)) {
                    const u32 co = wave_sum_u32_dpp(cov_o);
                    if (lane == 0) atomicAdd(&a.ctg[cur_c].cov_out, co);
                }
            }
            cov_o = 0; hbound = 0;
            return;
        }
        if (cur_c >= 0) {
            const bool narrow = !__any((sum_d | sum_d2) >> 50);
            const u64 s1 = narrow ? wave_sum_u56(sum_d) : wave_sum_u64(sum_d), s2 = narrow ? wave_sum_u56(sum_d2) : wave_sum_u64(sum_d2);
            const u32 c1 = wave_sum_u32_dpp(cov_w), c2 = wave_sum_u32_dpp(cov_f);
            const u32 m1 = wave_min_u32_dpp(mn), m2 = wave_max_u32_dpp(mx);
            DevContig *C = &a.ctg[cur_c];
            if (lane == 0) {
                if (s1) atomicAdd(&C->sum_d, s1);
                if (s2) atomicAdd(&C->sum_d2, s2);
                if (c1) atomicAdd(&C->cov_win, (u64)c1);
                if (c2) atomicAdd(&C->cov_full, (u64)c2);
                if (proc_win) {
                    atomicAdd(&C->proc_win, proc_win);
                    atomicMin(&C->min_d, m1);
                    atomicMax(&C->max_d, m2);
                }
            }
        }
        sum_d = sum_d2 = 0; proc_win = 0; cov_w = cov_f = 0; mn = 0xffffffffu; mx = 0;
    };
    auto load_runs = [&](const uint4 &d, uint2 &r0, uint2 &r1) {
        const u32 i0 = d.x + (u32)lane, i1 = i0 + 64u;
        r0 = i0 < d.y ? a.runs[i0] : make_uint2(0u, 0u);
        r1 = i1 < d.y ? a.runs[i1] : make_uint2(0u, 0u);
    };
    const u32 n_chunks = (n_tiles + chunk_tiles - 1) / chunk_tiles;
    if (wave_id >= n_chunks) return;
    u32 ch = wave_id;
    u32 t = ch * chunk_tiles, t_end = min(t + chunk_tiles, n_tiles);
    uint4 ds = a.desc[2 * (size_t)(a.tile_base + t)], dC1 = a.desc[2 * (size_t)(a.tile_base + t) + 1];
    uint2 rw0, rw1;
    load_runs(ds, rw0, rw1);
    for (;;) {
        u32 tn = t + 1, tn_end = t_end, chn = ch;
        bool chunk_end = false;
        if (tn >= t_end) {
            chunk_end = true;
            chn = ch + n_waves;
            tn = chn < n_chunks ? chn * chunk_tiles : 0xffffffffu;
            tn_end = chn < n_chunks ? min(tn + chunk_tiles, n_tiles) : 0u;
        }
        const bool have_next = tn != 0xffffffffu;
        uint4 nds = make_uint4(0u, 0u, 0u, 0u), ndC1 = make_uint4(0u, 0u, 0u, 0u);
        if (have_next) { nds = a.desc[2 * (size_t)(a.tile_base + tn)]; ndC1 = a.desc[2 * (size_t)(a.tile_base + tn) + 1]; }

        const u32 c = dC1.x, lo = dC1.y, L = ds.z, cxo = dC1.z, cxn = dC1.w;
        const bool live = (ds.x < ds.y || cxn != 0u) && !(ds.w & TILE_F_SLOW);
        uint4 sv0, sv1, ev0, ev1;
        if (live) {
            if ((int)c != cur_c) {
                flush();
                cur_c = (int)c;
                if (WANT_HIST) { hoff = a.ctg[c].hist_off; hcap = a.ctg[c].hist_cap; }
            }
            const u32 zb = TABLES == 2 ? 0u : 0x80008000u;
            const uint4 z4 = make_uint4(zb, zb, zb, zb);
            S4[2 * lane] = z4; S4[2 * lane + 1] = z4;
            if (TABLES == 2) { E4[2 * lane] = z4; E4[2 * lane + 1] = z4; }
            asm volatile("" ::: "memory");
            const u32 hi = lo + TW;
            auto add_run = [&](u32 s, u32 e) {
                if (s < hi && e > lo) {
                    const u32 s0 = s > lo ? s - lo : 0u;
                    atomicAdd(&S[s0 >> 1], (1u << DS) << ((s0 & 1u) << 4));
                    if (e < hi) {
                        const u32 e0 = e - lo;
                        if (TABLES == 2) atomicAdd(&E[e0 >> 1], 1u << ((e0 & 1u) << 4)); else atomicSub(&E[e0 >> 1], (1u << DS) << ((e0 & 1u) << 4));
                    }
                }
            };
            auto apply = [&](const uint2 rw, u32 i) {
                if (rw.y == 0u) return;
                const u32 type = rw.y >> 30;
                if (type <= RW_DOUBLE) {
                    const bool dbl = type == RW_DOUBLE;
                    const u32 l1 = dbl ? (rw.y & 1023u) : rw.y;
                    add_run(rw.x, rw.x + l1);
// ... 462 lines not shown
```

coverm_amd/csrc/prep_lean.hip.h:

```cpp
#pragma once
#include "pileup_kernels.hip.h"

namespace covk {

struct __attribute__((packed, aligned(4))) CigTriple { u32 a, b, c; };

__device__ __forceinline__ int dpp_prev(int v, int edge) { return __builtin_amdgcn_update_dpp(edge, v, 0x138, 0xf, 0xf, false); }
__device__ __forceinline__ int dpp_next(int v, int edge) { return __builtin_amdgcn_update_dpp(edge, v, 0x130, 0xf, 0xf, false); }

struct CigSum {
    u64 aligned, indel;
    u32 run_start, run_len, run2_start, run2_len, n_runs, span;
    bool oob, badcig, big;
};

__device__ __forceinline__ void cigar_sum3(u32 w0, u32 w1, u32 w2, int pos, u32 L, CigSum &o) {
    const u32 len0 = w0 >> 4, len1 = w1 >> 4, len2 = w2 >> 4;
    const u32 bit0 = 1u << (w0 & 15u), bit1 = 1u << (w1 & 15u), bit2 = 1u << (w2 & 15u);
    const bool m0 = (bit0 & 0x181u) != 0u, m1 = (bit1 & 0x181u) != 0u, m2 = (bit2 & 0x181u) != 0u;
    const u32 ref0 = (bit0 & 0x18du) ? len0 : 0u, ref1 = (bit1 & 0x18du) ? len1 : 0u, ref2 = (bit2 & 0x18du) ? len2 : 0u;
    const u32 c0 = (u32)pos, c1 = c0 + ref0, c2 = c1 + ref1;
    o.span = ref0 + ref1 + ref2;
    o.aligned = ((bit0 & 0x187u) ? len0 : 0u) + ((bit1 & 0x187u) ? len1 : 0u) + ((bit2 & 0x187u) ? len2 : 0u);
    o.indel = ((bit0 & 0x006u) ? len0 : 0u) + ((bit1 & 0x006u) ? len1 : 0u) + ((bit2 & 0x006u) ? len2 : 0u);
// ... 129 lines not shown
            const u32 al = (u32)cs.aligned;
            const float a = (float)al;
            survives = al >= h.min_aligned_length && a / (float)lsq >= h.min_aligned_percent &&
                       1.0f - (float)nmv32 / a >= h.min_percent_identity;
        }
    }
    const bool considered = survives && scan_gate;
    const bool masked_in = considered && tid_ok && mkv;
    u64 nmv = 0;
    double idv = 0.0;
    if (considered && !tid_ok) report_error(g, i, 7u);
    if (masked_in) {
        if (cs.badcig) report_error(g, i, 6u);
        else if (cs.oob) report_error(g, i, 4u);
        if (nk != 1u) report_error(g, i, nk == 0u ? 2u : 3u);
        else nmv = nmv32;
        if (WANT_IDENTITY && cs.aligned > 0) idv = ((double)cs.aligned - (double)nmv) / (double)cs.aligned;
    }
    bool is_bucket = false;
    if (in) {
        uint2 rw = make_uint2(0u, 0u);
        if (masked_in && cs.n_runs > 0) rw = run_word(cs, nops_all, is_bucket);
        h.runs[i] = rw;
        if (WANT_IDENTITY) {
            if (h.identn != nullptr) h.identn[i] = (masked_in && !supp) ? idv : 0.0;
            if (h.identp != nullptr) h.identp[i] = (masked_in && !supp && !sec) ? idv : 0.0;
        }
    }
    {
        const u64 qm = __ballot(is_bucket);
        if (qm != 0) {
            const int ql = __ffsll((long long)qm) - 1;
            u32 b = 0;
            if (lane == ql) b = atomicAdd(&g->n_cx, (u32)__popcll(qm));
            b = __builtin_amdgcn_readlane(b, ql);
            const u32 rank = __builtin_amdgcn_mbcnt_hi((u32)(qm >> 32), __builtin_amdgcn_mbcnt_lo((u32)qm, 0u));
            if (is_bucket && b + rank < cd.cx_list_cap) cd.cx_list[b + rank] = i;
        }
    }
    const bool tv = tid_ok && Lv > 0u;
    const u32 pc = pos < 0 ? 0u : min((u32)pos, Lv - 1u);
    const u32 tl = pc >> h.shift;
    const u32 key = t0v + tl;
    if (tv) {
        const bool same = pt == tid;
        const u32 pkey = t0v + ((ppos < 0 ? 0u : min((u32)ppos, Lv - 1u)) >> h.shift);
        if (!same || pkey != key) { atomicAdd(&h.tcnt[key], 0u - i); if (same) atomicAdd(&h.tcnt[pkey], i); }
        if (nt != tid) atomicAdd(&h.tcnt[key], i + 1u);
        const u32 e = cs.span > Lv - pc ? Lv : pc + cs.span;
        const u32 te = cs.span > 0u ? (e - 1u) >> h.shift : 0u;
        if (masked_in && cs.n_runs > 0u && cs.span > 0u && te > tl && !is_bucket)
            for (u32 t2 = tl + 1u; t2 <= te; t2++) atomicMin(&h.fov[t0v + t2], i);
    }
    const bool cnt = considered && tid_ok;
    const u64 cm = __ballot(cnt);
    {
        const u64 pm = __ballot(cnt && !(flag & 0x900u)), nsm = __ballot(cnt && !supp);
        const u32 nm_c = masked_in ? (u32)nmv : 0u, in_c = masked_in ? (u32)cs.indel : 0u, sp_c = masked_in ? cs.span : 0u;
        const bool wide = __any(masked_in && (nmv32 >= (1u << 25) || cs.indel >= (1ull << 25)));
        u32 r_np = 0, r_n = 0, r_nn = 0, r_sp = 0, r_first = 0, r_last = 0;
        u64 r_nm = 0, r_in = 0;
        u64 heads = 0;
        for (u64 todo = cm; todo != 0ull;) {
            const int fl = __builtin_ctzll(todo);
            const int t = __builtin_amdgcn_readlane(tid, fl);
            const bool mine = cnt && tid == t;
            const u64 m = __ballot(mine);
// ... 36 lines not shown
    u32 prim, pass, nons, first, last, span;
    u64 nm, indel;
    __device__ __forceinline__ void reset() { prim = pass = nons = 0; first = 0xffffffffu; last = 0; span = 0; nm = indel = 0; }
};

__device__ __forceinline__ void lean_flush(DevContig *ctg, int cur, LeanAcc &a) {
    if (cur >= 0 && a.pass) {
        const u32 span = wave_max_u32(a.span);
        const u64 nm = wave_sum_u64(a.nm), indel = wave_sum_u64(a.indel);
        if (lane_id() == 0) {
            DevContig *C = &ctg[cur];
            if (a.prim) atomicAdd(&C->n_primary, (u64)a.prim);
            atomicAdd(&C->n_pass, (u64)a.pass);
            if (a.nons) atomicAdd(&C->n_nonsupp, (u64)a.nons);
            if (nm) atomicAdd(&C->sum_nm, nm);
            if (indel) atomicAdd(&C->sum_indel, indel);
            if (span) atomicMax(&C->max_span, span);
            atomicMin(&C->first_rec, a.first);
            atomicMax(&C->last_rec, a.last);
        }
    }
    a.reset();
}

template <bool WANT_IDENTITY, bool FILTER, bool MASKED>
__device__ __forceinline__ void prep_lean_body(const PrepHot &h, const PrepArgs *__restrict__ pa) {
    __shared__ u32 blk_cnt[2][4];
    __shared__ u32 wmask[4];
    __shared__ PrepPartial wpart[4];
    const PrepCold *cold = &pa->cold;
    const int lane = lane_id();
    const u32 w = (u32)__builtin_amdgcn_readfirstlane((int)(threadIdx.x >> 6));
    const u32 wave_recs = h.steps * 64u;
    const u32 base = (blockIdx.x * 4u + w) * wave_recs;
    bool flushed_early = false;
    LeanAcc acc; acc.reset();
    int cur = -1;
    u32 g_prim = 0, g_cons = 0;
    u32 left_mask = 0;

    if (base < h.n) {
        const u32 nlast = h.n - 1u;
        const int *tid_w = h.tid + base; const int *pos_w = h.pos + base; const uint16_t *flag_w = h.flag + base;
        const uint8_t *nmk_w = h.nmk + base; const u32 *nm_w = h.nm + base; const u32 *coff_w = h.coff + base;
        const uint8_t *mapq_w = h.mapq + base; const u32 *lseq_w = h.lseq + base;
        uint2 *runs_w = h.runs + base;
        const u32 lmax = nlast - base;
        constexpr u32 LM = 0x1ffffu;

        int ptid_e = -2, ppos_e = 0;
        if (base > 0) { ptid_e = h.tid[base - 1u]; ppos_e = h.pos[base - 1u]; }
        u32 cur_L = 0, cur_t0 = 0, cur_mk = 1u;
        int td; u32 co0;
        { const u32 l = (u32)lane; td = tid_w[min(l, lmax) & LM]; co0 = coff_w[min(l, lmax + 1u) & LM]; }
        asm volatile("" : "+v"(td), "+v"(co0));

        for (u32 s = 0; s < h.steps; s++) {
            const u32 l0 = s * 64u, i0 = base + l0;
            if (i0 >= h.n) break;
            const u32 l = l0 + (u32)lane, i = i0 + (u32)lane;
            const u32 lc = min(l, lmax) & LM;
            const int tdn = tid_w[min(l + 64u, lmax) & LM];
            const u32 con = coff_w[min(l + 64u, lmax + 1u) & LM];
            const u32 flag = flag_w[lc];
            const int pos = pos_w[lc];
            const u32 nk = nmk_w[lc];
            const u32 nmv32 = nm_w[lc];
// ... 93 lines not shown
                    if (__builtin_expect(__all(!cross || te == tl + 1u), 1)) {
                        const u32 ckey = cross ? key : 0xfffffffeu;
                        const u32 pck = (u32)dpp_prev((int)ckey, (int)0xfffffffdu);
                        if (cross && ckey != pck) atomicMin(&h.fov[key + 1u], i);
                    } else if (cross) for (u32 t2 = tl + 1u; t2 <= te; t2++) atomicMin(&h.fov[t0c + t2], i);
                }
            }
            if (__builtin_expect(__any(ppos > pos), 0)) { if (lane == 0) atomicOr(&cold->ctg[tu].flags, F_POS_UNSORTED); }
            if (__builtin_expect(ntid_e != tu, 0)) { if (lane == 63) atomicMax(&cold->ctg[tu].rec_end, i + 1u); }
            const u64 cm = __ballot(considered);
            if (cm != 0ull) {
                g_cons += (u32)__popcll(cm);
                acc.prim += (u32)__popcll(__ballot(considered && !(flag & 0x900u)));
                acc.pass += (u32)__popcll(cm);
                acc.nons += (u32)__popcll(__ballot(considered && !supp));
                acc.first = min(acc.first, i0 + (u32)__builtin_ctzll(cm));
                acc.last = max(acc.last, i0 + 63u - (u32)__builtin_clzll(cm));
                if (masked_in) { acc.nm += nmv; acc.indel += cs.indel; acc.span = max(acc.span, cs.span); }
            }
            ptid_e = tu; ppos_e = __builtin_amdgcn_readlane(pos, 63);
            td = tdn; co0 = con;
        }
    }
    {
        PrepPartial pw;
        pw.tid = flushed_early ? -2 : cur;
        pw.prim = acc.prim; pw.pass = acc.pass; pw.nons = acc.nons;
        pw.span = wave_max_u32(acc.span); pw.first = acc.first; pw.last = acc.last;
        pw.nm = wave_sum_u64(acc.nm); pw.indel = wave_sum_u64(acc.indel); pw.pad = 0;
        if (lane == 0) wpart[w] = pw;
    }
    if (lane == 0) { blk_cnt[0][w] = g_prim; blk_cnt[1][w] = g_cons; wmask[w] = left_mask; }
    __syncthreads();
    if (w == 0u) {
        const u32 m0 = wmask[0], m1 = wmask[1], m2 = wmask[2], m3 = wmask[3];
        const u32 c0 = (u32)__popc(m0), c1 = c0 + (u32)__popc(m1), c2 = c1 + (u32)__popc(m2), total = c2 + (u32)__popc(m3);
        if (total) {
            u32 at = 0;
            if (lane == 0) at = atomicAdd(&cold->g->n_gen, total);
            at = (u32)__builtin_amdgcn_readfirstlane((int)at);
            for (u32 e = (u32)lane; e < total; e += 64u) {
                const u32 k = e < c0 ? 0u : e < c1 ? 1u : e < c2 ? 2u : 3u;
                u32 m = k == 0u ? m0 : k == 1u ? m1 : k == 2u ? m2 : m3;
                for (u32 r = e - (k == 0u ? 0u : k == 1u ? c0 : k == 2u ? c1 : c2); r != 0u; r--) m &= m - 1u;
                cold->gen_list[at + e] = (blockIdx.x * 4u + k) * wave_recs + (u32)__builtin_ctz(m) * 64u;
            }
        }
    }
    bool uniform_wg = true;
    {
        int t0 = -1;
        for (int k = 0; k < 4; k++) {
            const int t = wpart[k].tid;
            if (t == -2) uniform_wg = false;
            else if (t >= 0) { if (t0 < 0) t0 = t; else if (t != t0) uniform_wg = false; }
        }
        if (threadIdx.x == 0) {
            PrepPartial o; o.tid = -1; o.prim = o.pass = o.nons = o.span = 0; o.first = 0xffffffffu; o.last = 0; o.pad = 0; o.nm = o.indel = 0;
            if (uniform_wg && t0 >= 0) {
                o.tid = t0;
                for (int k = 0; k < 4; k++) {
                    const PrepPartial &q = wpart[k];
                    if (q.tid < 0) continue;
                    o.prim += q.prim; o.pass += q.pass; o.nons += q.nons; o.span = max(o.span, q.span);
                    o.first = min(o.first, q.first); o.last = max(o.last, q.last); o.nm += q.nm; o.indel += q.indel;
                }
            }
            cold->part[blockIdx.x] = o;
        }
    }
    if (!uniform_wg) lean_flush(cold->ctg, cur, acc);
    if (threadIdx.x == 0) {
        const u32 p = blk_cnt[0][0] + blk_cnt[0][1] + blk_cnt[0][2] + blk_cnt[0][3];
        const u32 c = blk_cnt[1][0] + blk_cnt[1][1] + blk_cnt[1][2] + blk_cnt[1][3];
        const u32 slot = (blockIdx.x % COUNTER_SLOTS) * 8u;
        DevGlobal *g = cold->g;
        if (p) atomicAdd(&g->prim_slots[slot], (u64)p);
        if (c) atomicAdd(&g->cons_slots[slot], (u64)c);
    }
}

template <bool WANT_IDENTITY, bool FILTER, bool MASKED>
__global__ __launch_bounds__(256) __attribute__((amdgpu_waves_per_eu(8, 8))) void k_prep_lean(PrepHot h, const PrepArgs *__restrict__ pa) {
    prep_lean_body<WANT_IDENTITY, FILTER, MASKED>(h, pa);
}
template <bool WANT_IDENTITY, bool FILTER, bool MASKED>
__global__ __launch_bounds__(256) void k_prep_generic(const PrepArgs *__restrict__ pa, u32 all_steps) {
    const u32 n = all_steps ? all_steps : pa->cold.g->n_gen;
    const u32 *__restrict__ list = pa->cold.gen_list;
    for (u32 j = blockIdx.x * 4u + (threadIdx.x >> 6); j < n; j += gridDim.x * 4u) {
        const u32 i0 = all_steps ? j * 64u : (u32)__builtin_amdgcn_readfirstlane((int)list[j]);
        GenFields f;
        gen_load<FILTER>(pa->hot, i0, f);
        prep_step_generic<WANT_IDENTITY, FILTER, MASKED>(pa, i0, f);
    }
}

}
```

coverm_amd/engine.py:

```python
import ctypes as C
from dataclasses import dataclass
from typing import Optional

import numpy as np

from . import native
from .native import CovBatch, CovConfig, CovError, CovSummary


@dataclass
class RecordBatch:
    tid: np.ndarray
    pos: np.ndarray
    flag: np.ndarray
    mapq: np.ndarray
    nm: np.ndarray
    nm_kind: np.ndarray
    l_seq: np.ndarray
    cigar_off: np.ndarray
    cigar: np.ndarray

    @property
    def n_records(self):
        return int(self.tid.shape[0])
# ... 217 lines not shown
    def group_kernel_ms(self):
        ms = C.c_double(0)
        n = C.c_uint32(0)
        self._check(self._lib.cov_kernel_ms(self._h, native.K_GROUP, C.byref(ms), C.byref(n)))
        return ms.value, n.value

    def sam_ingest(self, path_or_fileobj, mates=False, group=False):
        from . import bam
        return bam.sam_ingest(self, path_or_fileobj, want_mates=mates, group=group)

    def sam_kernel_ms(self):
        ms = C.c_double(0)
        n = C.c_uint32(0)
        self._check(self._lib.cov_kernel_ms(self._h, native.K_SAM, C.byref(ms), C.byref(n)))
        return ms.value, n.value

    def store_spills(self):
        return int(self._lib.cov_store_spills(self._h))

    def kernel_ms(self):
        out = {}
        for k, name in native.KERNEL_NAMES.items():
            ms = C.c_double(0)
            n = C.c_uint32(0)
            self._check(self._lib.cov_kernel_ms(self._h, k, C.byref(ms), C.byref(n)))
            out[name] = (ms.value, n.value)
        return out

    def last_paths(self):
        v = (C.c_uint32 * 4)()
        self._check(self._lib.cov_last_paths(self._h, C.byref(v)))
        return dict(listed_steps=int(v[0]), generic_only=bool(v[1]), slow_tiles=int(v[2]), bucket_records=int(v[3]))

    def algorithmic_bytes(self):
        b = C.c_uint64(0)
        self._check(self._lib.cov_algorithmic_bytes(self._h, C.byref(b)))
        return int(b.value)
```

coverm_amd/native.py:

```python
import ctypes as C
import os

import numpy as np

_HERE = os.path.dirname(os.path.abspath(__file__))
LIB_PATH = os.path.join(_HERE, "libcovermhip.so")

COV_OK = 0
ERR_UNSORTED, ERR_NM_MISSING, ERR_NM_BADTYPE, ERR_POS_OOB, ERR_BAD_CIGAR, ERR_BAD_TID = 1, 2, 3, 4, 6, 7
ERR_INVALID_ARG, ERR_HIP, ERR_STATE = 16, 17, 18
WANT_HIST, WANT_IDENTITY = 1, 2
WANT_IDENTITY_PRIMARY_ONLY, WANT_IDENTITY_NONSUPP_ONLY = 4, 8
K_PREP, K_RANGES, K_PILEUP, K_IDENTITY, K_HIST, K_HIST_COMPACT, K_ESTIMATE, K_COUNT = 0, 1, 2, 3, 4, 5, 6, 11
K_GENOME = 7
K_GROUP = 8
K_SEP = 10
K_SAM = 9
KERNEL_NAMES = {K_PREP: "k_prep", K_RANGES: "k_ranges", K_PILEUP: "k_pileup", K_IDENTITY: "k_identity",
                K_HIST: "k_hist", K_HIST_COMPACT: "k_hist_compact", K_ESTIMATE: "k_estimate"}


class CovConfig(C.Structure):
    _fields_ = [("device", C.c_int32), ("include_improper_pairs", C.c_uint8), ("include_supplementary", C.c_uint8),
                ("include_secondary", C.c_uint8), ("filter_single", C.c_uint8), ("min_mapq", C.c_uint8),
                ("reserved0", C.c_uint8 * 3), ("min_aligned_length", C.c_uint32),
                ("min_percent_identity", C.c_float), ("min_aligned_percent", C.c_float),
                ("contig_end_exclusion", C.c_uint64), ("want", C.c_uint32), ("reserved1", C.c_uint32)]


class CovBatch(C.Structure):
    _fields_ = [("tid", C.c_void_p), ("pos", C.c_void_p), ("flag", C.c_void_p), ("mapq", C.c_void_p),
                ("nm", C.c_void_p), ("nm_kind", C.c_void_p), ("l_seq", C.c_void_p), ("cigar_off", C.c_void_p),
                ("cigar", C.c_void_p), ("n_records", C.c_uint64)]


class CovSummary(C.Structure):
    _fields_ = [("num_detected_primary_alignments", C.c_uint64), ("n_records", C.c_uint64),
                ("n_considered", C.c_uint64), ("hist_total", C.c_uint64)]


CONTIG_STATS_DTYPE = np.dtype([
    ("n_primary", "<u8"), ("n_pass", "<u8"), ("n_nonsupp", "<u8"), ("sum_nm", "<u8"), ("sum_indel", "<u8"),
    ("sum_identity_primary", "<f8"), ("sum_identity_nonsupp", "<f8"), ("win_sum_d", "<u8"), ("win_sum_d2", "<u8"),
    ("win_covered", "<u8"), ("full_covered", "<u8"), ("first_record", "<u8"), ("last_record", "<u8"),
    ("win_min_d", "<u4"), ("win_max_d", "<u4"), ("hist_len", "<u4"), ("reserved", "<u4"), ("hist_off", "<u8")])
assert CONTIG_STATS_DTYPE.itemsize == 128

GENOME_STATS_DTYPE = np.dtype([("reads_in_genome", "<u8"), ("genome_len", "<u8"), ("n_contigs_seen", "<u4"), ("any_nonzero", "<u4")])
assert GENOME_STATS_DTYPE.itemsize == 24

GENOME_ENTRY_DTYPE = np.dtype([("reads", "<u8"), ("first_tid", "<u4"), ("gid", "<i4"), ("n_contigs_seen", "<u4"), ("any_nonzero", "<u4")])
assert GENOME_ENTRY_DTYPE.itemsize == 24

EXPORTS = ["cov_abi_version", "cov_create", "cov_destroy", "cov_last_error", "cov_set_targets",
           "cov_set_target_mask", "cov_push_batch", "cov_push_batch_device", "cov_finish", "cov_fetch_hist",
           "cov_copy_depth", "cov_reset", "cov_kernel_ms", "cov_algorithmic_bytes", "cov_last_paths",
           "cov_set_genomes", "cov_finish_genomes", "cov_fetch_genome_estimates", "cov_fetch_genome_stats",
           "cov_set_genome_runs", "cov_genome_entry_count", "cov_fetch_genome_entries",
           "cov_sam_begin", "cov_sam_window_bytes", "cov_sam_slot_wait", "cov_sam_feed", "cov_sam_end"]

_lib = None


class NativeLibraryMissing(RuntimeError):
    pass


def _torch_hip_first():
    import sys
    t = sys.modules.get("torch")
    if t is None:
        return
    try:
        if t.cuda.is_available():
            t.cuda.init()
    except Exception:
        pass


def lib():
    global _lib
    if _lib is not None:
        return _lib
    if not os.path.exists(LIB_PATH):
        raise NativeLibraryMissing(
            "%s not found — build it with `python -m coverm_amd.build` (hipcc, gfx950). "
            "coverm_amd has no CPU fallback for the coverage hot path." % LIB_PATH)
    _torch_hip_first()
    L = C.CDLL(LIB_PATH)
    L.cov_abi_version.restype = C.c_int
    L.cov_last_error.restype = C.c_char_p
    L.cov_last_error.argtypes = [C.c_void_p]
    L.cov_create.argtypes = [C.POINTER(CovConfig), C.POINTER(C.c_void_p)]
    L.cov_destroy.argtypes = [C.c_void_p]
    L.cov_destroy.restype = None
    L.cov_set_targets.argtypes = [C.c_void_p, C.c_uint32, C.c_void_p]
    L.cov_set_target_mask.argtypes = [C.c_void_p, C.c_void_p]
    L.cov_push_batch.argtypes = [C.c_void_p, C.POINTER(CovBatch)]
    L.cov_push_batch_device.argtypes = [C.c_void_p, C.POINTER(CovBatch)]
    L.cov_finish.argtypes = [C.c_void_p, C.c_void_p, C.POINTER(CovSummary)]
    L.cov_fetch_hist.argtypes = [C.c_void_p, C.c_void_p]
    L.cov_copy_depth.argtypes = [C.c_void_p, C.c_uint32, C.c_void_p]
    L.cov_reset.argtypes = [C.c_void_p]
    L.cov_kernel_ms.argtypes = [C.c_void_p, C.c_int, C.POINTER(C.c_double), C.POINTER(C.c_uint32)]
    L.cov_algorithmic_bytes.argtypes = [C.c_void_p, C.POINTER(C.c_uint64)]
    L.cov_last_paths.argtypes = [C.c_void_p, C.POINTER(C.c_uint32 * 4)]
    L.cov_set_estimators.argtypes = [C.c_void_p, C.c_void_p, C.c_uint32]
    L.cov_fetch_estimates.argtypes = [C.c_void_p, C.c_void_p]
    L.cov_set_genomes.argtypes = [C.c_void_p, C.c_void_p, C.c_uint32]
    L.cov_finish_genomes.argtypes = [C.c_void_p, C.POINTER(CovSummary)]
    L.cov_fetch_genome_estimates.argtypes = [C.c_void_p, C.c_void_p]
    L.cov_fetch_genome_stats.argtypes = [C.c_void_p, C.c_void_p]
    L.cov_set_genome_runs.argtypes = [C.c_void_p, C.c_void_p, C.c_uint32]
    L.cov_genome_entry_count.argtypes = [C.c_void_p, C.POINTER(C.c_uint32)]
    L.cov_fetch_genome_entries.argtypes = [C.c_void_p, C.c_void_p]
    L.cov_store_spills.argtypes = [C.c_void_p]
    L.cov_store_spills.restype = C.c_uint32
    L.cov_group_records.argtypes = [C.c_void_p, C.POINTER(C.c_uint64)]
    L.cov_ingest_want_grouping.argtypes = [C.c_void_p, C.c_int]
    _lib = L
    return L


class CovError(RuntimeError):
    def __init__(self, status, message):
        super().__init__("covermhip status %d: %s" % (status, message))
        self.status = status
        self.message = message
```

include/covermhip.h:

```cpp
#ifndef COVERMHIP_H
#define COVERMHIP_H

#include <stddef.h>
#include <stdint.h>

#ifdef __cplusplus
extern "C" {
#endif

#define COVERMHIP_ABI_VERSION 1

typedef struct cov_session cov_session;

typedef enum {
    COV_OK = 0,
    COV_ERR_UNSORTED = 1,
    COV_ERR_NM_MISSING = 2,
    COV_ERR_NM_BADTYPE = 3,
    COV_ERR_POS_OOB = 4,
    COV_ERR_BAD_CIGAR = 6,
    COV_ERR_BAD_TID = 7,
    COV_ERR_INVALID_ARG = 16,
    COV_ERR_HIP = 17,
    COV_ERR_STATE = 18,
// ... 112 lines not shown
cov_status cov_ingest_feed(cov_session *s, int slot, const void *host_bytes, uint64_t file_offset, uint64_t n_bytes,
                           const cov_bgzf_block *blocks, uint32_t n_blocks);
cov_status cov_ingest_end(cov_session *s, uint64_t *n_records);
cov_status cov_ingest_abort(cov_session *s);
cov_status cov_ingest_release(cov_session *s);
cov_status cov_ingest_copy_inflated(cov_session *s, uint64_t offset, uint64_t n, void *out);
cov_status cov_sam_begin(cov_session *s, const char *names_blob, const uint64_t *name_off, uint32_t n_names, uint64_t expected_bytes);
uint64_t cov_sam_window_bytes(const cov_session *s);
cov_status cov_sam_slot_wait(cov_session *s, int slot);
cov_status cov_sam_feed(cov_session *s, int slot, const void *host_bytes, uint64_t n_bytes);
cov_status cov_sam_end(cov_session *s, uint64_t *n_records);
typedef struct {
    int32_t filter_single;
    uint8_t min_mapq;
    uint8_t pad[3];
    uint32_t min_aligned_length_single;
    float min_percent_identity_single, min_aligned_percent_single;
    uint32_t min_aligned_length_pair;
    float min_percent_identity_pair, min_aligned_percent_pair;
} cov_pair_filter;
cov_status cov_ingest_want_mates(cov_session *s, int on);
cov_status cov_pair_filter_apply(cov_session *s, const cov_pair_filter *f, uint64_t *n_selected, uint64_t *n_primary);
cov_status cov_ingest_want_grouping(cov_session *s, int on);
cov_status cov_group_records(cov_session *s, uint64_t *n_moved);
cov_status cov_copy_records(cov_session *s, const cov_batch *host, uint64_t *n_records, uint64_t *n_cigar);
cov_status cov_copy_mates(cov_session *s, int32_t *mtid, uint64_t *qh1, uint32_t *qh2);

cov_status cov_gather(cov_session *const *sessions, uint32_t n, uint32_t root);
cov_status cov_gathered(cov_session *root_session, uint32_t rank, cov_contig_stats *stats, cov_summary *summary);

cov_status cov_kernel_ms(const cov_session *s, cov_kernel_id k, double *ms_total, uint32_t *launches);
typedef struct { uint32_t listed_steps, generic_only, slow_tiles, bucket_records; } cov_path_counts;
cov_status cov_last_paths(const cov_session *s, cov_path_counts *out);
cov_status cov_algorithmic_bytes(const cov_session *s, uint64_t *bytes);

typedef struct {
    int32_t kind;
    float min_fraction_covered_bases;
    uint64_t contig_end_exclusion;
    int32_t exclude_mismatches;
    float trim_min, trim_max;
} cov_estimator;
#define COV_EST_MEAN 0
#define COV_EST_TRIMMED_MEAN 1
#define COV_EST_PILEUP_COUNTS 2
#define COV_EST_COVERED_FRACTION 3
#define COV_EST_COVERED_BASES 4
#define COV_EST_RPKM 5
#define COV_EST_TPM 6
#define COV_EST_VARIANCE 7
#define COV_EST_LENGTH 8
#define COV_EST_READ_COUNT 9
#define COV_EST_READS_PER_BASE 10
#define COV_EST_ANIR 11
#define COV_EST_MAX 16
cov_status cov_set_estimators(cov_session *s, const cov_estimator *est, uint32_t n_est);
cov_status cov_fetch_estimates(cov_session *s, float *out);

typedef struct {
    uint64_t reads_in_genome;
    uint64_t genome_len;
    uint32_t n_contigs_seen;
    uint32_t any_nonzero;
} cov_genome_stats;
cov_status cov_set_genomes(cov_session *s, const int32_t *genome_of_tid, uint32_t n_genomes);
cov_status cov_finish_genomes(cov_session *s, cov_summary *summary);
// ... 40 lines not shown
```

Baseline: 50.42 billion.

## Split finish pipeline at a record cut and overlap halves on two streams

Splits the finish pass at a record cut point into parts A and B. Part A's prep, scan and pileup run on the main stream while part B's run on a side stream, synchronised through events and a device-side cut structure. The goal is to overlap the kernel chains of the two halves so the GPU stays busy through launch gaps and tail effects. In exchange it adds duplicate scan buffers, more events, a fallback path and an extra finish retry, plus the risk of the two halves contending for the same device.

```diff
diff --git a/coverm_amd/csrc/covermhip.hip b/coverm_amd/csrc/covermhip.hip
--- a/coverm_amd/csrc/covermhip.hip
+++ b/coverm_amd/csrc/covermhip.hip
@@ -28,6 +28,7 @@
 #include "knobs.h"
 #include "record_store.h"
 #include "store_plan_core.h"
+#include "finish_split_core.h"
 
 using namespace covk;
 
@@ -225,6 +226,16 @@
     hipEvent_t ev[COV_K_COUNT][2] = {};
     hipEvent_t ev_begin[COV_K_COUNT] = {};
     int ev_fresh = -1;
+    long long split_knob = -1;
+    bool split_fell_back = false;
+    bool last_split = false;
+    uint32_t last_split_r1 = 0, last_split_contig = 0;
+    hipEvent_t ev_b[COV_K_COUNT][2] = {}, ev_begin_b[COV_K_COUNT] = {};
+    int ev_fresh_b = -1;
+    bool k_in_b[COV_K_COUNT] = {};
+    hipEvent_t ev_a_lean = nullptr, ev_a_prep = nullptr, ev_a_layout = nullptr, ev_b_done = nullptr;
+    hipEvent_t ev_tail[2] = {};
+    DevBuf<u32> d_tscan_b, d_ttop_b, d_cx_scan_b, d_cx_top_b;
     float k_ms[COV_K_COUNT] = {};
     uint32_t k_launches[COV_K_COUNT] = {};
 };
@@ -327,14 +338,33 @@
     for (int k = 0; k < COV_K_COUNT; k++)
         for (int j = 0; j < 2; j++) (void)hipEventCreate(&s->ev[k][j]);
 }
-void time_begin(cov_session *s, int k) {
+void time_begin(cov_session *s, int k, int lane = 0) {
+    if (lane) {
+        if (s->ev_fresh_b >= 0) { s->ev_begin_b[k] = s->ev_b[s->ev_fresh_b][1]; return; }
+        (void)hipEventRecord(s->ev_b[k][0], s->side); s->ev_begin_b[k] = s->ev_b[k][0];
+        return;
+    }
     if (s->ev_fresh >= 0) { s->ev_begin[k] = s->ev[s->ev_fresh][1]; return; }
     (void)hipEventRecord(s->ev[k][0], s->stream); s->ev_begin[k] = s->ev[k][0];
 }
-void time_end(cov_session *s, int k) { (void)hipEventRecord(s->ev[k][1], s->stream); s->k_launches[k]++; s->ev_fresh = k; }
+void time_end(cov_session *s, int k, int lane = 0) {
+    if (lane) { (void)hipEventRecord(s->ev_b[k][1], s->side); s->k_launches[k]++; s->ev_fresh_b = k; s->k_in_b[k] = true; return; }
+    (void)hipEventRecord(s->ev[k][1], s->stream); s->k_launches[k]++; s->ev_fresh = k;
+}
+hipError_t split_events(cov_session *s) {
+    if (s->ev_b_done) return hipSuccess;
+    for (int k : {COV_K_PREP, COV_K_RANGES, COV_K_HIST, COV_K_PILEUP})
+        for (int j = 0; j < 2; j++) { const hipError_t e = hipEventCreate(&s->ev_b[k][j]); if (e != hipSuccess) return e; }
+    for (int j = 0; j < 2; j++) { const hipError_t e = hipEventCreate(&s->ev_tail[j]); if (e != hipSuccess) return e; }
+    for (hipEvent_t *e : {&s->ev_a_lean, &s->ev_a_prep, &s->ev_a_layout, &s->ev_b_done}) {
+        const hipError_t r = hipEventCreateWithFlags(e, hipEventDisableTiming);
+        if (r != hipSuccess) return r;
+    }
+    return hipSuccess;
+}
 
 template <bool H, int TABLES>
-void launch_fast_v(cov_session *s, const PileupArgs &a, u32 n_tiles) {
+void launch_fast_v(cov_session *s, const PileupArgs &a, u32 n_tiles, hipStream_t st) {
     const auto kern = TABLES == 1 ? &k_pileup_fast<H> : &k_pileup_fast2t<H>;
     const size_t smem = pileup_fast_smem_bytes(H, TABLES == 1 ? FAST_HB : FAST_HB7, TABLES);
     static std::atomic<int> occ_dev[64];
@@ -353,12 +383,12 @@
     }
     const u32 wg_per_cu = 8u * (u32)occ;
     const u32 grid = std::max(1u, std::min((n_chunks + 3) / 4, (u32)s->n_cus * wg_per_cu));
-    hipLaunchKernelGGL(kern, dim3(grid), dim3(256), smem, s->stream, a, n_tiles, chunk);
+    hipLaunchKernelGGL(kern, dim3(grid), dim3(256), smem, st, a, n_tiles, chunk);
 }
 template <bool H>
-void launch_fast_t(cov_session *s, const PileupArgs &a, u32 n_tiles) {
-    if (s->fast_tables == 2) launch_fast_v<H, 2>(s, a, n_tiles);
-    else launch_fast_v<H, 1>(s, a, n_tiles);
+void launch_fast_t(cov_session *s, const PileupArgs &a, u32 n_tiles, hipStream_t st) {
+    if (s->fast_tables == 2) launch_fast_v<H, 2>(s, a, n_tiles, st);
+    else launch_fast_v<H, 1>(s, a, n_tiles, st);
 }
 
 template <bool H, bool W>
@@ -391,7 +421,7 @@
 template <bool H, bool W>
 void launch_any_pileup(cov_session *s, const PileupArgs &a, u32 n_tiles) {
     if (s->use_fast && !W) {
-        launch_fast_t<H>(s, a, n_tiles);
+        launch_fast_t<H>(s, a, n_tiles, s->stream);
         launch_stream_t<H, W>(s, a, n_tiles, true);
     } else launch_stream_t<H, W>(s, a, n_tiles);
 }
@@ -478,6 +508,7 @@
     { long long v; if (covknob::get("store_cap_records", v) && v >= 1) s->cap_records = std::min<uint64_t>((uint64_t)v, 0xfffffff0ull); }
     { long long v; if (covknob::get("store_cap_cigar", v) && v >= 1) s->cap_cigar = std::min<uint64_t>((uint64_t)v, 0xfffffff0ull); }
     { long long v; if (covknob::get("pileup_chunk_tiles", v) && v >= 1 && v <= 64) s->chunk_tiles = (int)v; }
+    { long long v; if (covknob::get("finish_split_records", v) && v >= 0) s->split_knob = v; }
     e = hipEventCreateWithFlags(&s->ev_prep_done, hipEventDisableTiming);
     if (e == hipSuccess) e = hipEventCreateWithFlags(&s->ev_side_done, hipEventDisableTiming);
     if (e == hipSuccess) e = hipStreamCreateWithFlags(&s->stream, hipStreamNonBlocking);
@@ -511,6 +542,7 @@
     s->d_stop_cnt.release(); s->d_stop_seg.release(); s->d_sent.release();
     s->d_gout.release(); if (s->h_gout) (void)hipHostFree(s->h_gout); s->h_gout = nullptr;
     s->d_tile_first.release(); s->d_tcnt.release(); s->d_fov.release(); s->d_tscan.release(); s->d_ttop.release(); s->d_slow_list.release();
+    s->d_tscan_b.release(); s->d_ttop_b.release(); s->d_cx_scan_b.release(); s->d_cx_top_b.release();
     s->d_ctg_scratch.release(); s->d_depth_all.release(); s->d_depth_off.release(); s->d_iv.release(); s->d_ivst.release(); s->d_ivhist.release();
     s->d_cx_list.release(); s->d_cx_cnt.release(); s->d_cx_cur.release(); s->d_cx_scan.release(); s->d_cx_top.release(); s->d_cx_runs.release();
     if (s->side) {
@@ -553,7 +585,8 @@
     if (s->ev_prep_done) (void)hipEventDestroy(s->ev_prep_done);
     if (s->ev_side_done) (void)hipEventDestroy(s->ev_side_done); s->d_arena.release(); s->d_chist.release(); s->d_depth.release();
     for (int k = 0; k < COV_K_COUNT; k++)
-        for (int j = 0; j < 2; j++) if (s->ev[k][j]) (void)hipEventDestroy(s->ev[k][j]);
+        for (int j = 0; j < 2; j++) { if (s->ev[k][j]) (void)hipEventDestroy(s->ev[k][j]); if (s->ev_b[k][j]) (void)hipEventDestroy(s->ev_b[k][j]); }
+    for (hipEvent_t e : {s->ev_a_lean, s->ev_a_prep, s->ev_a_layout, s->ev_b_done, s->ev_tail[0], s->ev_tail[1]}) if (e) (void)hipEventDestroy(e);
     if (s->stream) (void)hipStreamDestroy(s->stream);
     delete s;
 }
@@ -785,6 +818,7 @@
     }
     s->adopted = false; s->store.n_records = 0; s->store.n_cigar = 0; s->finished = false; s->depth_all_valid = false; s->store.mates_valid = 0; s->ing_was_span = false;
     s->spill.clear(); s->merged_valid = false; s->merged_hist.clear(); s->ing_rec_spilled = 0; s->spill_retry_at = 0; s->spill_est.clear(); s->est_valid = false; s->gen_valid = false;
+    s->split_fell_back = false;
     return COV_OK;
 }
 
@@ -927,6 +961,7 @@
     bool again = false;
     cov_status st = finish_once(s, stats, summary, again);
     if (st == COV_OK && again) st = finish_once(s, stats, summary, again);
+    if (st == COV_OK && again) st = finish_once(s, stats, summary, again);
     if (st == COV_OK && again) { s->err = "internal error: bucket sizing did not converge"; return COV_ERR_STATE; }
     return st;
 }
@@ -1005,8 +1040,37 @@
     f.min_percent_identity = s->cfg.min_percent_identity; f.min_aligned_percent = s->cfg.min_aligned_percent;
     double *idp = (want_id && !(s->cfg.want & COV_WANT_IDENTITY_NONSUPP_ONLY)) ? s->d_identp.p : nullptr;
     double *idn = (want_id && !(s->cfg.want & COV_WANT_IDENTITY_PRIMARY_ONLY)) ? s->d_ident.p : nullptr;
-    HIPCHK(s->d_prep_args.reserve(1, st));
+    static_assert(256 * 2 * PREP_PASSES == fsplit::WG_RECORDS, "the cut is a multiple of k_prep_lean's workgroup");
+    fsplit::Plan sp{false, 0, 0, 0};
+    if (R && s->n_tiles) {
+        const fsplit::Route rt{prep_kernel == 7, long_cigars, s->use_fast, s->in_spill || s->spill.active, want_id, lean, s->split_fell_back};
+        sp = fsplit::plan(R, nT, rt, s->split_knob);
+    }
+    const bool split = sp.split;
+    const u32 R1 = split ? (u32)sp.r1 : 0u, blocks_a = (u32)sp.blocks_a, blocks_b = (u32)sp.blocks_b;
+    s->last_split = split; s->last_split_r1 = R1; s->last_split_contig = 0;
+    for (int k = 0; k < COV_K_COUNT; k++) s->k_in_b[k] = false;
+    s->ev_fresh_b = -1;
+    bool tail_timed = false;
+    hipStream_t sb = nullptr;
+    const u32 n_scan_blocks = (s->n_tiles + 1023u) / 1024u;
+    if (split) {
+        if (!s->side) {
+            (void)ingest_prep_wait(s);
+            if (s->ing_aux && !s->ing_active) s->side = s->ing_aux;
+            else { HIPCHK(hipStreamCreateWithFlags(&s->side, hipStreamNonBlocking)); s->side_owned = true; }
+        }
+        sb = s->side;
+        HIPCHK(split_events(s));
+        HIPCHK(s->d_tscan_b.reserve(s->n_tiles, st)); HIPCHK(s->d_ttop_b.reserve((size_t)n_scan_blocks + 2, st));
+        HIPCHK(s->d_cx_scan_b.reserve(s->n_tiles, st)); HIPCHK(s->d_cx_top_b.reserve((size_t)n_scan_blocks + 2, st));
+        HIPCHK(s->d_cx_list.reserve(2 * (size_t)cx.list_cap, st));
+        cx.list = s->d_cx_list.p;
+    }
+    HIPCHK(s->d_prep_args.reserve(2, st));
     HIPCHK(s->d_gen_list.reserve((size_t)R / 64 + 2, st));
+    DevGlobal *const dg = s->d_glob.p;
+    const PartRef pr_all{&dg->cut, PART_ALL, 0}, pr_a{&dg->cut, PART_A, 0}, pr_b{&dg->cut, PART_B, 0};
     PrepArgs pa{};
     {
         PrepHot &ph = pa.hot;
@@ -1017,12 +1081,23 @@
         ph.p1_mask = 0x4u | (f.include_secondary ? 0u : 0x100u) | (f.include_supplementary ? 0u : 0x800u);
         ph.min_mapq = f.min_mapq; ph.min_aligned_length = f.min_aligned_length; ph.min_percent_identity = f.min_percent_identity; ph.min_aligned_percent = f.min_aligned_percent;
         PrepCold &pc = pa.cold;
-        pc.ctg = s->d_ctg.p; pc.g = s->d_glob.p; pc.part = s->d_part.p; pc.cx_list = cx.list; pc.mask = mask; pc.tlen = s->d_tlen.p; pc.tile_first = s->d_tile_first.p;
-        pc.cx_list_cap = cx.list_cap; pc.gen_list = s->d_gen_list.p;
-    }
-    hipLaunchKernelGGL(k_init, dim3((std::max(std::max(nT, COUNTER_SLOTS * 8), s->n_tiles) + 255) / 256), dim3(256), 0, st, s->d_ctg.p,
-                       nT, s->d_glob.p, ti, cx, s->d_prep_args.p, pa);
+        pc.ctg = s->d_ctg.p; pc.g = dg; pc.part = s->d_part.p; pc.cx_list = cx.list; pc.mask = mask; pc.tlen = s->d_tlen.p; pc.tile_first = s->d_tile_first.p;
+        pc.cx_list_cap = cx.list_cap; pc.gen_list = s->d_gen_list.p; pc.n_gen = &dg->n_gen; pc.n_cx = &dg->n_cx; pc.blk0 = 0;
+    }
+    u32 *const cx_list_b = split ? cx.list + cx.list_cap : nullptr;
+    {
+        const SplitInit si{r.tid, split ? s->d_gen_list.p + R1 / 64u : nullptr, cx_list_b, R1, blocks_a};
+        hipLaunchKernelGGL(k_init, dim3((std::max(std::max(nT, COUNTER_SLOTS * 8), s->n_tiles) + 255) / 256), dim3(256), 0, st, s->d_ctg.p,
+                           nT, dg, ti, cx, s->d_prep_args.p, pa, si);
+    }
     HIPCHK(hipGetLastError());
+    const CxWork cw_all{{cx.list, nullptr}, {&dg->n_cx, nullptr}, &dg->cx_total, pr_all};
+    const CxWork cw_a_cnt{{cx.list, nullptr}, {&dg->n_cx, nullptr}, &dg->cut.cx_total_a, pr_all};
+    const CxWork cw_a_fill{{cx.list, nullptr}, {&dg->n_cx, nullptr}, &dg->cut.cx_total_a, pr_a};
+    const CxWork cw_b_cnt{{cx_list_b, nullptr}, {&dg->cut.n_cx_b, nullptr}, &dg->cx_total, pr_b};
+    const CxWork cw_b_fill{{cx.list, cx_list_b}, {&dg->n_cx, &dg->cut.n_cx_b}, &dg->cx_total, pr_b};
+    CxIdx cx_b = cx;
+    if (split) { cx_b.cscan = s->d_cx_scan_b.p; cx_b.ctop = s->d_cx_top_b.p; }
 
     if (R) {
         time_begin(s, COV_K_PREP);
@@ -1030,19 +1105,19 @@
         const bool gen_all = prep_kernel != 7 && (uint64_t)R < (uint64_t)nT * 128u;
         s->last_gen_all = gen_all;
         const u32 gen_grid = gen_all ? std::min<u32>((u32)s->n_cus * 64u, (n_steps + 3u) / 4u) : std::min<u32>((u32)s->n_cus * 8u, (n_steps + 3u) / 4u);
+        auto launch_prep = [&](int what, hipStream_t pst, const PrepHot &hot, const PrepArgs *pap, u32 grid) {
 #define COV_LAUNCH_PREP(ID, FI, MA)                                                                                                       \
         do {                                                                                                                              \
             if (prep_kernel == 7)                                                                                                         \
-                hipLaunchKernelGGL((k_prep7s<ID, FI, MA>), dim3(prep_grid), dim3(256), 0, st, r, s->d_tlen.p, nT, mask, f, s->d_ctg.p,   \
+                hipLaunchKernelGGL((k_prep7s<ID, FI, MA>), dim3(prep_grid), dim3(256), 0, pst, r, s->d_tlen.p, nT, mask, f, s->d_ctg.p,  \
                                    s->d_glob.p, s->d_runs.p, idp, idn, s->d_part.p, ti, prep_passes, prep_b, cx.list, cx.list_cap);      \
             else if (gen_all)                                                                                                             \
-                hipLaunchKernelGGL((k_prep_generic<ID, FI, MA>), dim3(gen_grid), dim3(256), 0, st, (const PrepArgs *)s->d_prep_args.p, n_steps); \
+                hipLaunchKernelGGL((k_prep_generic<ID, FI, MA>), dim3(gen_grid), dim3(256), 0, pst, pap, n_steps);                       \
             else {                                                                                                                        \
-                hipLaunchKernelGGL((k_prep_lean<ID, FI, MA>), dim3(prep_grid), dim3(256), 0, st, pa.hot, (const PrepArgs *)s->d_prep_args.p); \
-                hipLaunchKernelGGL((k_prep_generic<ID, FI, MA>), dim3(gen_grid), dim3(256), 0, st, (const PrepArgs *)s->d_prep_args.p, 0u); \
+                if (what != 2) hipLaunchKernelGGL((k_prep_lean<ID, FI, MA>), dim3(grid), dim3(256), 0, pst, hot, pap);                   \
+                if (what != 1) hipLaunchKernelGGL((k_prep_generic<ID, FI, MA>), dim3(gen_grid), dim3(256), 0, pst, pap, 0u);             \
             }                                                                                                                             \
         } while (0)
-        {
             const int key = (want_id ? 4 : 0) | (s->cfg.filter_single ? 2 : 0) | (mask != nullptr ? 1 : 0);
             switch (key) {
             case 0: COV_LAUNCH_PREP(false, false, false); break;
@@ -1054,14 +1129,33 @@
             case 6: COV_LAUNCH_PREP(true, true, false); break;
             default: COV_LAUNCH_PREP(true, true, true); break;
             }
-        }
 #undef COV_LAUNCH_PREP
-        if (nT) {
-            const u32 n_red = gen_all ? 0u : (nT + 3u) / 4u, cx_grid0 = (u32)s->n_cus * 8u;
-            hipLaunchKernelGGL(k_post_prep, dim3(n_red + cx_grid0), dim3(256), 0, st, r, s->d_tlen.p, s->d_glob.p, cx, ti, s->d_ctg.p, nT, (const PrepPartial *)s->d_part.p,
-                               prep_grid, prep_chunk, n_red);
-        }
-        time_end(s, COV_K_PREP);
+        };
+        const u32 n_red = gen_all ? 0u : (nT + 3u) / 4u, cx_grid0 = (u32)s->n_cus * 8u;
+        auto launch_post_prep = [&](hipStream_t pst, const CxWork &cw, const CxIdx &pcx, u32 n_parts, const PartRef &red) {
+            hipLaunchKernelGGL(k_post_prep, dim3(n_red + cx_grid0), dim3(256), 0, pst, r, s->d_tlen.p, cw, pcx, ti, s->d_ctg.p, nT, (const PrepPartial *)s->d_part.p,
+                               n_parts, prep_chunk, n_red, red);
+        };
+        const PrepArgs *pa_dev = s->d_prep_args.p;
+        if (!split) {
+            launch_prep(0, st, pa.hot, pa_dev, prep_grid);
+            if (nT) launch_post_prep(st, cw_all, cx, prep_grid, pr_all);
+            time_end(s, COV_K_PREP);
+        } else {
+            launch_prep(1, st, pa.hot, pa_dev, blocks_a);
+            HIPCHK(hipEventRecord(s->ev_a_lean, st));
+            launch_prep(2, st, pa.hot, pa_dev, 0);
+            HIPCHK(hipEventRecord(s->ev_a_prep, st));
+            launch_post_prep(st, cw_a_cnt, cx, blocks_a, pr_a);
+            time_end(s, COV_K_PREP);
+            HIPCHK(hipStreamWaitEvent(sb, s->ev_a_lean, 0));
+            time_begin(s, COV_K_PREP, 1);
+            launch_prep(1, sb, pa.hot, pa_dev + 1, blocks_b);
+            launch_prep(2, sb, pa.hot, pa_dev + 1, 0);
+            HIPCHK(hipStreamWaitEvent(sb, s->ev_a_prep, 0));
+            launch_post_prep(sb, cw_b_cnt, cx_b, prep_grid, pr_b);
+            time_end(s, COV_K_PREP, 1);
+        }
         HIPCHK(hipGetLastError());
         if (want_id && nT) {
             if (!s->side) {
@@ -1088,56 +1182,96 @@
         }
     }
     if (R && s->n_tiles) {
-        time_begin(s, COV_K_RANGES);
-        const u32 n_blocks = (s->n_tiles + 1023u) / 1024u;
+        const u32 n_blocks = n_scan_blocks;
         const u32 cx_grid = (u32)s->n_cus * 8u;
-        ScanPair sp{};
-        sp.cnt[0] = s->d_tcnt.p; sp.scan[0] = s->d_tscan.p; sp.top[0] = s->d_ttop.p; sp.total[0] = nullptr;
-        sp.cnt[1] = s->d_cx_cnt.p; sp.scan[1] = s->d_cx_scan.p; sp.top[1] = s->d_cx_top.p; sp.total[1] = &s->d_glob.p->cx_total;
-        hipLaunchKernelGGL(k_tile_scan1, dim3(2u * n_blocks), dim3(1024), 0, st, sp, s->n_tiles, n_blocks);
-        hipLaunchKernelGGL(k_tile_scan2, dim3(2), dim3(1024), 0, st, sp, n_blocks);
-        hipLaunchKernelGGL((k_cx_expand<true>), dim3(cx_grid), dim3(256), 0, st, r, s->d_tlen.p, s->d_glob.p, cx, ti);
         u32 *slow_list = s->use_fast ? s->d_slow_list.p : nullptr;
-        if (want_hist)
-            hipLaunchKernelGGL((k_ranges<true>), dim3((s->n_tiles + 255) / 256), dim3(256), 0, st, s->d_tile_contig.p,
-                               s->d_tile_start.p, s->n_tiles, s->d_tlen.p, mask, s->d_ctg.p, s->d_desc.p, ti, s->d_tscan.p,
-                               s->d_ttop.p, cx, s->d_glob.p, slow_list);
-        else
-            hipLaunchKernelGGL((k_ranges<false>), dim3((s->n_tiles + 255) / 256), dim3(256), 0, st, s->d_tile_contig.p,
-                               s->d_tile_start.p, s->n_tiles, s->d_tlen.p, mask, s->d_ctg.p, s->d_desc.p, ti, s->d_tscan.p,
-                               s->d_ttop.p, cx, s->d_glob.p, slow_list);
-        time_end(s, COV_K_RANGES);
-        HIPCHK(hipGetLastError());
-        if (want_hist) {
-            time_begin(s, COV_K_HIST);
-            const u32 hb = (nT + 1023u) / 1024u;
-            HIPCHK(s->d_hist_top.reserve(hb, st));
-            hipLaunchKernelGGL((k_hist_sum<0>), dim3(hb), dim3(1024), 0, st, (const DevContig *)s->d_ctg.p, nT, s->d_tlen.p, mask, (u64)s->cfg.contig_end_exclusion, s->d_hist_top.p);
-            hipLaunchKernelGGL((k_hist_off<0>), dim3(hb), dim3(1024), 0, st, s->d_ctg.p, nT, s->d_tlen.p, mask, (u64)s->cfg.contig_end_exclusion, (const u64 *)s->d_hist_top.p, s->d_glob.p);
-            hipLaunchKernelGGL(k_zero_u32, dim3(2048), dim3(256), 0, st, s->d_arena.p, &s->d_glob.p->hist_cap_total);
-            time_end(s, COV_K_HIST);
-            HIPCHK(hipGetLastError());
-        }
+        const u32 hb = (nT + 1023u) / 1024u;
+        if (want_hist) HIPCHK(s->d_hist_top.reserve((size_t)hb * (split ? 2u : 1u), st));
+        auto launch_ranges = [&](hipStream_t pst, int lane, const PartRef &pr, const CxWork &fill, const CxIdx &pcx, u32 *tscan, u32 *ttop, u32 *cscan, u32 *ctop, u64 *cx_total) {
+            time_begin(s, COV_K_RANGES, lane);
+            ScanPair scp{};
+            scp.cnt[0] = s->d_tcnt.p; scp.scan[0] = tscan; scp.top[0] = ttop; scp.total[0] = nullptr;
+            scp.cnt[1] = s->d_cx_cnt.p; scp.scan[1] = cscan; scp.top[1] = ctop; scp.total[1] = cx_total;
+            hipLaunchKernelGGL(k_tile_scan1, dim3(2u * n_blocks), dim3(1024), 0, pst, scp, s->n_tiles, n_blocks);
+            hipLaunchKernelGGL(k_tile_scan2, dim3(2), dim3(1024), 0, pst, scp, n_blocks);
+            hipLaunchKernelGGL((k_cx_expand<true>), dim3(cx_grid), dim3(256), 0, pst, r, s->d_tlen.p, fill, pcx, ti);
+            if (want_hist)
+                hipLaunchKernelGGL((k_ranges<true>), dim3((s->n_tiles + 255) / 256), dim3(256), 0, pst, s->d_tile_contig.p,
+                                   s->d_tile_start.p, s->n_tiles, s->d_tlen.p, mask, s->d_ctg.p, s->d_desc.p, ti, tscan,
+                                   ttop, pcx, dg, slow_list, pr, (const u64 *)cx_total);
+            else
+                hipLaunchKernelGGL((k_ranges<false>), dim3((s->n_tiles + 255) / 256), dim3(256), 0, pst, s->d_tile_contig.p,
+                                   s->d_tile_start.p, s->n_tiles, s->d_tlen.p, mask, s->d_ctg.p, s->d_desc.p, ti, tscan,
+                                   ttop, pcx, dg, slow_list, pr, (const u64 *)cx_total);
+            time_end(s, COV_K_RANGES, lane);
+        };
+        auto launch_layout = [&](hipStream_t pst, int lane, const PartRef &pr, u64 *top, const u64 *zero_lo, const u64 *zero_hi) {
+            time_begin(s, COV_K_HIST, lane);
+            hipLaunchKernelGGL((k_hist_sum<0>), dim3(hb), dim3(1024), 0, pst, (const DevContig *)s->d_ctg.p, nT, s->d_tlen.p, mask, (u64)s->cfg.contig_end_exclusion, top, pr);
+            hipLaunchKernelGGL((k_hist_off<0>), dim3(hb), dim3(1024), 0, pst, s->d_ctg.p, nT, s->d_tlen.p, mask, (u64)s->cfg.contig_end_exclusion, (const u64 *)top, dg, pr);
+            if (pr.part == PART_A) (void)hipEventRecord(s->ev_a_layout, pst);
+            hipLaunchKernelGGL(k_zero_u32, dim3(2048), dim3(256), 0, pst, s->d_arena.p, zero_lo, zero_hi);
+            time_end(s, COV_K_HIST, lane);
+        };
         PileupArgs a = pileup_args(s);
         compacted = want_hist && (s->est.n == 0 || s->hist_fetch_seen);
         derive_in_est = want_hist && !compacted && !(s->have_mask || s->have_runs) && s->est.n != 0;
-        time_begin(s, COV_K_PILEUP);
-        if (want_hist) launch_any_pileup<true, false>(s, a, s->n_tiles);
-        else launch_any_pileup<false, false>(s, a, s->n_tiles);
-        if (want_hist && !derive_in_est) {
-            if (est_lanes) hipLaunchKernelGGL((k_hist_stats<true>), dim3((nT + 255) / 256), dim3(256), 0, st, s->d_ctg.p, nT, (const u32 *)s->d_tlen.p, mask, (u64)s->cfg.contig_end_exclusion, (const u32 *)s->d_arena.p);
-            else hipLaunchKernelGGL((k_hist_stats<false>), dim3((nT + 3) / 4), dim3(256), 0, st, s->d_ctg.p, nT, (const u32 *)s->d_tlen.p, mask, (u64)s->cfg.contig_end_exclusion, (const u32 *)s->d_arena.p);
-        }
-        time_end(s, COV_K_PILEUP);
-        HIPCHK(hipGetLastError());
+        auto launch_hist_stats = [&]() {
+            if (want_hist && !derive_in_est) {
+                if (est_lanes) hipLaunchKernelGGL((k_hist_stats<true>), dim3((nT + 255) / 256), dim3(256), 0, st, s->d_ctg.p, nT, (const u32 *)s->d_tlen.p, mask, (u64)s->cfg.contig_end_exclusion, (const u32 *)s->d_arena.p);
+                else hipLaunchKernelGGL((k_hist_stats<false>), dim3((nT + 3) / 4), dim3(256), 0, st, s->d_ctg.p, nT, (const u32 *)s->d_tlen.p, mask, (u64)s->cfg.contig_end_exclusion, (const u32 *)s->d_arena.p);
+            }
+        };
+        if (!split) {
+            launch_ranges(st, 0, pr_all, cw_all, cx, s->d_tscan.p, s->d_ttop.p, s->d_cx_scan.p, s->d_cx_top.p, &dg->cx_total);
+            HIPCHK(hipGetLastError());
+            if (want_hist) {
+                launch_layout(st, 0, pr_all, s->d_hist_top.p, nullptr, &dg->hist_cap_total);
+                HIPCHK(hipGetLastError());
+            }
+            time_begin(s, COV_K_PILEUP);
+            if (want_hist) launch_any_pileup<true, false>(s, a, s->n_tiles);
+            else launch_any_pileup<false, false>(s, a, s->n_tiles);
+            launch_hist_stats();
+            time_end(s, COV_K_PILEUP);
+            HIPCHK(hipGetLastError());
+        } else {
+            launch_ranges(st, 0, pr_a, cw_a_fill, cx, s->d_tscan.p, s->d_ttop.p, s->d_cx_scan.p, s->d_cx_top.p, &dg->cut.cx_total_a);
+            if (want_hist) launch_layout(st, 0, pr_a, s->d_hist_top.p, nullptr, &dg->cut.arena_a);
+            a.cut = &dg->cut; a.part = PART_A;
+            time_begin(s, COV_K_PILEUP);
+            if (want_hist) launch_fast_t<true>(s, a, s->n_tiles, st); else launch_fast_t<false>(s, a, s->n_tiles, st);
+            time_end(s, COV_K_PILEUP);
+            HIPCHK(hipGetLastError());
+            launch_ranges(sb, 1, pr_b, cw_b_fill, cx_b, s->d_tscan_b.p, s->d_ttop_b.p, s->d_cx_scan_b.p, s->d_cx_top_b.p, &dg->cx_total);
+            if (want_hist) {
+                HIPCHK(hipStreamWaitEvent(sb, s->ev_a_layout, 0));
+                s->ev_fresh_b = -1;
+                launch_layout(sb, 1, pr_b, s->d_hist_top.p + hb, &dg->cut.arena_a, &dg->hist_cap_total);
+            }
+            a.part = PART_B;
+            time_begin(s, COV_K_PILEUP, 1);
+            if (want_hist) launch_fast_t<true>(s, a, s->n_tiles, sb); else launch_fast_t<false>(s, a, s->n_tiles, sb);
+            time_end(s, COV_K_PILEUP, 1);
+            HIPCHK(hipGetLastError());
+            HIPCHK(hipEventRecord(s->ev_b_done, sb));
+            HIPCHK(hipStreamWaitEvent(st, s->ev_b_done, 0));
+            a.part = PART_ALL;
+            (void)hipEventRecord(s->ev_tail[0], st);
+            if (want_hist) launch_stream_t<true, false>(s, a, s->n_tiles, true); else launch_stream_t<false, false>(s, a, s->n_tiles, true);
+            launch_hist_stats();
+            (void)hipEventRecord(s->ev_tail[1], st);
+            s->k_launches[COV_K_PILEUP]++; tail_timed = true; s->ev_fresh = -1;
+            HIPCHK(hipGetLastError());
+        }
         if (want_hist) {
             s->hist_prefetched = 0;
             if (compacted) {
                 HIPCHK(s->d_chist.reserve((size_t)R + nT + 1, st));
                 time_begin(s, COV_K_HIST_COMPACT);
                 const u32 hb = (nT + 1023u) / 1024u;
-                hipLaunchKernelGGL((k_hist_sum<1>), dim3(hb), dim3(1024), 0, st, (const DevContig *)s->d_ctg.p, nT, s->d_tlen.p, mask, (u64)s->cfg.contig_end_exclusion, s->d_hist_top.p);
-                hipLaunchKernelGGL((k_hist_off<1>), dim3(hb), dim3(1024), 0, st, s->d_ctg.p, nT, s->d_tlen.p, mask, (u64)s->cfg.contig_end_exclusion, (const u64 *)s->d_hist_top.p, s->d_glob.p);
+                hipLaunchKernelGGL((k_hist_sum<1>), dim3(hb), dim3(1024), 0, st, (const DevContig *)s->d_ctg.p, nT, s->d_tlen.p, mask, (u64)s->cfg.contig_end_exclusion, s->d_hist_top.p, pr_all);
+                hipLaunchKernelGGL((k_hist_off<1>), dim3(hb), dim3(1024), 0, st, s->d_ctg.p, nT, s->d_tlen.p, mask, (u64)s->cfg.contig_end_exclusion, (const u64 *)s->d_hist_top.p, s->d_glob.p, pr_all);
                 hipLaunchKernelGGL(k_hist_compact, dim3((nT + 3u) / 4u), dim3(256), 0, st, s->d_ctg.p, nT, s->d_tlen.p, (u64)s->cfg.contig_end_exclusion, s->d_arena.p, s->d_chist.p);
                 time_end(s, COV_K_HIST_COMPACT);
                 HIPCHK(hipGetLastError());
@@ -1270,8 +1404,20 @@
         again = true;
         return COV_OK;
     }
+    if (split) {
+        const u32 c_cut = std::min(s->h_glob.cut.c_cut, nT);
+        s->last_split_contig = c_cut;
+        bool behind = false;
+        for (u32 c = 0; c < c_cut && !behind; c++) behind = s->h_ctg[c].rec_start < s->h_ctg[c].rec_end && s->h_ctg[c].rec_end > R1;
+        if (behind) { s->split_fell_back = true; again = true; return COV_OK; }
+    }
     for (int k = 0; k < COV_K_COUNT; k++)
-        if (s->k_launches[k]) (void)hipEventElapsedTime(&s->k_ms[k], k == COV_K_IDENTITY ? s->ev[k][0] : s->ev_begin[k], s->ev[k][1]);
+        if (s->k_launches[k]) {
+            (void)hipEventElapsedTime(&s->k_ms[k], k == COV_K_IDENTITY ? s->ev[k][0] : s->ev_begin[k], s->ev[k][1]);
+            float more = 0.f;
+            if (s->k_in_b[k] && hipEventElapsedTime(&more, s->ev_begin_b[k], s->ev_b[k][1]) == hipSuccess) s->k_ms[k] += more;
+            if (k == COV_K_PILEUP && tail_timed && hipEventElapsedTime(&more, s->ev_tail[0], s->ev_tail[1]) == hipSuccess) s->k_ms[k] += more;
+        }
 
     {
         const uint64_t ncig = s->adopted ? s->adopted_ncig : s->store.n_cigar;
@@ -2410,8 +2556,8 @@
         const uint8_t *mask = s->have_mask ? (const uint8_t *)s->d_mask.p : (const uint8_t *)nullptr;
         const u32 hb = (s->n_targets + 1023u) / 1024u;
         HIPCHK(s->d_hist_top.reserve(hb, s->stream));
-        hipLaunchKernelGGL((k_hist_sum<1>), dim3(hb), dim3(1024), 0, s->stream, (const DevContig *)s->d_ctg.p, s->n_targets, s->d_tlen.p, mask, (u64)s->cfg.contig_end_exclusion, s->d_hist_top.p);
-        hipLaunchKernelGGL((k_hist_off<1>), dim3(hb), dim3(1024), 0, s->stream, s->d_ctg.p, s->n_targets, s->d_tlen.p, mask, (u64)s->cfg.contig_end_exclusion, (const u64 *)s->d_hist_top.p, s->d_glob.p);
+        hipLaunchKernelGGL((k_hist_sum<1>), dim3(hb), dim3(1024), 0, s->stream, (const DevContig *)s->d_ctg.p, s->n_targets, s->d_tlen.p, mask, (u64)s->cfg.contig_end_exclusion, s->d_hist_top.p, PartRef{&s->d_glob.p->cut, PART_ALL, 0});
+        hipLaunchKernelGGL((k_hist_off<1>), dim3(hb), dim3(1024), 0, s->stream, s->d_ctg.p, s->n_targets, s->d_tlen.p, mask, (u64)s->cfg.contig_end_exclusion, (const u64 *)s->d_hist_top.p, s->d_glob.p, PartRef{&s->d_glob.p->cut, PART_ALL, 0});
         hipLaunchKernelGGL(k_hist_compact, dim3((s->n_targets + 3u) / 4u), dim3(256), 0, s->stream, s->d_ctg.p, s->n_targets, s->d_tlen.p,
                            (u64)s->cfg.contig_end_exclusion, s->d_arena.p, s->d_chist.p);
         HIPCHK(hipGetLastError());
@@ -2539,8 +2685,15 @@
 
 cov_status cov_last_paths(const cov_session *s, cov_path_counts *out) {
     if (!s || !out) return COV_ERR_INVALID_ARG;
-    out->listed_steps = s->h_glob.n_gen; out->generic_only = s->last_gen_all ? 1u : 0u;
-    out->slow_tiles = s->h_glob.n_slow; out->bucket_records = s->h_glob.n_cx;
+    out->listed_steps = s->h_glob.n_gen + s->h_glob.cut.n_gen_b; out->generic_only = s->last_gen_all ? 1u : 0u;
+    out->slow_tiles = s->h_glob.n_slow; out->bucket_records = s->h_glob.n_cx + s->h_glob.cut.n_cx_b;
+    return COV_OK;
+}
+
+cov_status cov_last_split(const cov_session *s, cov_split_info *out) {
+    if (!s || !out) return COV_ERR_INVALID_ARG;
+    out->split = s->last_split ? 1u : 0u; out->fell_back = s->split_fell_back ? 1u : 0u;
+    out->cut_record = s->last_split_r1; out->cut_contig = s->last_split_contig;
     return COV_OK;
 }
 
diff --git a/coverm_amd/csrc/finish_split_core.h b/coverm_amd/csrc/finish_split_core.h
--- /dev/null
+++ b/coverm_amd/csrc/finish_split_core.h
@@ -0,0 +1,36 @@
+#pragma once
+
+namespace fsplit {
+typedef unsigned long long u64;
+constexpr u64 WG_RECORDS = 4096;
+constexpr u64 MIN_RECORDS_PER_TARGET = 128;
+constexpr u64 AUTO_FLOOR = 0;
+
+struct Route {
+    bool prep7, long_cigars, use_fast, in_spill, identity, lean, fell_back;
+};
+struct Plan {
+    bool split;
+    u64 r1;
+    u64 blocks_a, blocks_b;
+};
+
+inline Plan plan(u64 R, u64 n_targets, const Route &rt, long long knob) {
+    Plan p{false, 0, 0, 0};
+    const u64 blocks = (R + WG_RECORDS - 1) / WG_RECORDS;
+    if (knob == 0 || R >= 0xfffffff0ull) return p;
+    if (rt.prep7 || rt.long_cigars || !rt.use_fast || rt.in_spill || rt.identity || rt.lean || rt.fell_back) return p;
+    if (n_targets == 0 || R < n_targets * MIN_RECORDS_PER_TARGET) return p;
+    u64 r1;
+    if (knob > 0) {
+        r1 = (((u64)knob + WG_RECORDS / 2) / WG_RECORDS) * WG_RECORDS;
+        if (r1 == 0) r1 = WG_RECORDS;
+    } else {
+        if (AUTO_FLOOR == 0 || R < AUTO_FLOOR) return p;
+        r1 = (blocks / 2) * WG_RECORDS;
+    }
+    if (r1 == 0 || r1 >= R) return p;
+    p.split = true; p.r1 = r1; p.blocks_a = r1 / WG_RECORDS; p.blocks_b = blocks - p.blocks_a;
+    return p;
+}
+}
diff --git a/coverm_amd/csrc/pileup_kernels.hip.h b/coverm_amd/csrc/pileup_kernels.hip.h
--- a/coverm_amd/csrc/pileup_kernels.hip.h
+++ b/coverm_amd/csrc/pileup_kernels.hip.h
@@ -35,6 +35,19 @@
 static_assert(sizeof(DevContig) == 160, "DevContig layout");
 
 constexpr u32 COUNTER_SLOTS = 64;
+struct SplitCut {
+    u32 c_cut, tile_cut;
+    u64 arena_a;
+    u64 cx_total_a;
+    u32 n_cx_b, n_gen_b;
+    u32 r1, pad;
+};
+constexpr u32 PART_ALL = 0, PART_A = 1, PART_B = 2;
+struct PartRef {
+    SplitCut *cut; u32 part, pad;
+    __device__ __forceinline__ bool contig_in(u32 c) const { return part == PART_ALL || (part == PART_A ? c < cut->c_cut : c >= cut->c_cut); }
+    __device__ __forceinline__ bool tile_in(u32 t) const { return part == PART_ALL || (part == PART_A ? t < cut->tile_cut : t >= cut->tile_cut); }
+};
 struct DevGlobal {
     u64 first_error;
     u64 hist_cap_total;
@@ -47,8 +60,10 @@
     u64 pad2[2];
     u64 prim_slots[COUNTER_SLOTS * 8];
     u64 cons_slots[COUNTER_SLOTS * 8];
-    u32 pad_q[8 * 16];
+    SplitCut cut;
+    u32 pad_q[8 * 16 - sizeof(SplitCut) / 4];
 };
+static_assert(sizeof(SplitCut) == 40, "SplitCut layout");
 
 struct FilterCfg {
     u32 include_improper_pairs, include_supplementary, include_secondary;
@@ -154,7 +169,9 @@
     DevContig *ctg; DevGlobal *g; PrepPartial *part; u32 *cx_list;
     const uint8_t *mask; const u32 *tlen; const u32 *tile_first;
     u32 *gen_list;
-    u32 cx_list_cap, pad;
+    u32 *n_gen, *n_cx;
+    u32 cx_list_cap;
+    u32 blk0;
 };
 struct PrepHot {
     const int32_t *tid, *pos;
@@ -174,9 +191,26 @@
 };
 struct PrepArgs { PrepHot hot; PrepCold cold; };
 
-__global__ void k_init(DevContig *ctg, u32 n_targets, DevGlobal *g, TileIdx ti, CxIdx cx, PrepArgs *pa_out, PrepArgs pa) {
+struct SplitInit { const int32_t *tid; u32 *gen_list_b, *cx_list_b; u32 r1, blk0_b; };
+__global__ void k_init(DevContig *ctg, u32 n_targets, DevGlobal *g, TileIdx ti, CxIdx cx, PrepArgs *pa_out, PrepArgs pa, SplitInit si) {
     u32 c = blockIdx.x * blockDim.x + threadIdx.x;
-    if (c == 0 && pa_out != nullptr) *pa_out = pa;
+    if (c == 0 && pa_out != nullptr) {
+        pa_out[0] = pa;
+        if (si.r1) {
+            pa.cold.blk0 = si.blk0_b; pa.cold.gen_list = si.gen_list_b; pa.cold.cx_list = si.cx_list_b;
+            pa.cold.n_gen = &g->cut.n_gen_b; pa.cold.n_cx = &g->cut.n_cx_b;
+            pa_out[1] = pa;
+        }
+    }
+    if (c == 0) {
+        SplitCut k;
+        k.c_cut = n_targets; k.tile_cut = ti.n_tiles; k.arena_a = 0; k.cx_total_a = 0; k.n_cx_b = 0; k.n_gen_b = 0; k.r1 = si.r1; k.pad = 0;
+        if (si.r1) {
+            const int t = si.tid[si.r1 - 1u];
+            if (t >= 0 && (u32)t < n_targets) { k.c_cut = (u32)t; k.tile_cut = ti.tile_first[t]; }
+        }
+        g->cut = k;
+    }
     if (c < ti.n_tiles) { ti.tcnt[c] = 0u; ti.fov[c] = 0xffffffffu; cx.cnt[c] = 0u; cx.cur[c] = 0u; }
     if (c == 0) {
         g->first_error = ~0ull; g->hist_cap_total = 0; g->chist_total = 0; g->internal_error = 0;
@@ -668,8 +702,9 @@
 COV_PREP_KERNEL(k_prep7s, __attribute__((amdgpu_waves_per_eu(7, 7))), true, 1)
 #undef COV_PREP_KERNEL
 
-__device__ __forceinline__ void prep_reduce_body(u32 c, DevContig *ctg, u32 n_targets, const PrepPartial *__restrict__ part, u32 n_parts, u32 chunk_recs) {
-    if (c >= n_targets) return;
+__device__ __forceinline__ void prep_reduce_body(u32 c, DevContig *ctg, u32 n_targets, const PrepPartial *__restrict__ part, u32 n_parts, u32 chunk_recs,
+                                                 const PartRef &pr) {
+    if (c >= n_targets || !pr.contig_in(c)) return;
     DevContig *C = &ctg[c];
     const u32 rs = C->rec_start, re = C->rec_end;
     if (rs >= re) return;
@@ -740,15 +775,16 @@
     if (total != nullptr && threadIdx.x == 0) *total = carry_s;
 }
 
+struct CxWork { const u32 *list[2]; const u32 *n[2]; const u64 *total; PartRef pr; };
 template <bool FILL>
-__device__ __forceinline__ void cx_expand_body(const Records &r, const u32 *__restrict__ tlen, DevGlobal *g, const CxIdx &cx, const TileIdx &ti, u32 wave, u32 n_waves) {
+__device__ __forceinline__ void cx_expand_list(const Records &r, const u32 *__restrict__ tlen, const CxIdx &cx, const TileIdx &ti, const u32 *__restrict__ list, u32 n,
+                                               const PartRef &pr, u32 wave, u32 n_waves) {
     const int lane = lane_id();
-    const u32 n = min(g->n_cx, cx.list_cap);
-    if (FILL && g->cx_total > cx.runs_cap) return;
     const u64 lt = lane == 0 ? 0ull : (~0ull >> (64 - lane));
     for (u32 j = wave; j < n; j += n_waves) {
-        const u32 i = cx.list[j];
+        const u32 i = list[j];
         const int tid = r.tid[i];
+        if (!pr.contig_in((u32)tid)) continue;
         const u32 co0 = r.cigar_off[i], nops = r.cigar_off[i + 1] - co0;
         const u32 L = tlen[tid], t0 = ti.tile_first[tid];
         long long cur0 = r.pos[i];
@@ -786,16 +822,22 @@
         }
     }
 }
-
 template <bool FILL>
-__global__ __launch_bounds__(256) void k_cx_expand(Records r, const u32 *__restrict__ tlen, DevGlobal *g, CxIdx cx, TileIdx ti) {
-    cx_expand_body<FILL>(r, tlen, g, cx, ti, blockIdx.x * 4u + (threadIdx.x >> 6), gridDim.x * 4u);
-}
-
-__global__ __launch_bounds__(256) void k_post_prep(Records r, const u32 *__restrict__ tlen, DevGlobal *g, CxIdx cx, TileIdx ti, DevContig *ctg, u32 n_targets,
-                                                   const PrepPartial *__restrict__ part, u32 n_parts, u32 chunk_recs, u32 n_red) {
-    if (blockIdx.x < n_red) prep_reduce_body(blockIdx.x * 4u + (threadIdx.x >> 6), ctg, n_targets, part, n_parts, chunk_recs);
-    else cx_expand_body<false>(r, tlen, g, cx, ti, (blockIdx.x - n_red) * 4u + (threadIdx.x >> 6), (gridDim.x - n_red) * 4u);
+__device__ __forceinline__ void cx_expand_body(const Records &r, const u32 *__restrict__ tlen, const CxWork &cw, const CxIdx &cx, const TileIdx &ti, u32 wave, u32 n_waves) {
+    if (FILL && *cw.total > cx.runs_cap) return;
+    for (int k = 0; k < 2; k++)
+        if (cw.list[k] != nullptr) cx_expand_list<FILL>(r, tlen, cx, ti, cw.list[k], min(*cw.n[k], cx.list_cap), cw.pr, wave, n_waves);
+}
+
+template <bool FILL>
+__global__ __launch_bounds__(256) void k_cx_expand(Records r, const u32 *__restrict__ tlen, CxWork cw, CxIdx cx, TileIdx ti) {
+    cx_expand_body<FILL>(r, tlen, cw, cx, ti, blockIdx.x * 4u + (threadIdx.x >> 6), gridDim.x * 4u);
+}
+
+__global__ __launch_bounds__(256) void k_post_prep(Records r, const u32 *__restrict__ tlen, CxWork cw, CxIdx cx, TileIdx ti, DevContig *ctg, u32 n_targets,
+                                                   const PrepPartial *__restrict__ part, u32 n_parts, u32 chunk_recs, u32 n_red, PartRef red) {
+    if (blockIdx.x < n_red) prep_reduce_body(blockIdx.x * 4u + (threadIdx.x >> 6), ctg, n_targets, part, n_parts, chunk_recs, red);
+    else cx_expand_body<false>(r, tlen, cw, cx, ti, (blockIdx.x - n_red) * 4u + (threadIdx.x >> 6), (gridDim.x - n_red) * 4u);
 }
 
 template <bool WANT_HIST>
@@ -803,19 +845,21 @@
                                                 u32 n_tiles, const u32 *__restrict__ tlen, const uint8_t *__restrict__ mask,
                                                 DevContig *ctg, uint4 *__restrict__ desc, TileIdx ti,
                                                 const u32 *__restrict__ tscan, const u32 *__restrict__ ttop, CxIdx cx,
-                                                DevGlobal *__restrict__ g, u32 *__restrict__ slow_list) {
+                                                DevGlobal *__restrict__ g, u32 *__restrict__ slow_list, PartRef pr, const u64 *__restrict__ cx_total) {
     const u32 t = blockIdx.x * blockDim.x + threadIdx.x;
-    if (t >= n_tiles) return;
+    if (t >= n_tiles || !pr.tile_in(t)) return;
     const u32 c = tile_contig[t];
     DevContig *C = &ctg[c];
     uint4 out = make_uint4(0u, 0u, tlen[c], 0u);
     u32 cxn = 0, cxo = 0;
     if (C->n_pass != 0 && (mask == nullptr || mask[c])) {
-        const u32 rs = C->rec_start, re = C->rec_end;
-        cxn = g->cx_total <= cx.runs_cap ? cx.cnt[t] : 0u;
+        u32 rs = C->rec_start, re = C->rec_end;
+        cxn = *cx_total <= cx.runs_cap ? cx.cnt[t] : 0u;
         cxo = cx.cscan[t] + cx.ctop[t >> 10];
-        if (C->n_groups != 1u) out.w = 1u;
-        if (C->n_groups != 1u || (C->flags & F_POS_UNSORTED)) {
+        bool generic = C->n_groups != 1u;
+        if (pr.part == PART_A && re > pr.cut->r1) { re = pr.cut->r1; rs = min(rs, re); generic = true; }
+        if (generic) out.w = 1u;
+        if (generic || (C->flags & F_POS_UNSORTED)) {
             out.x = rs; out.y = re;
         } else {
             const u32 tf = ti.tile_first[c];
@@ -867,36 +911,39 @@
 }
 template <int MODE>
 __global__ __launch_bounds__(1024) void k_hist_sum(const DevContig *__restrict__ ctg, u32 n_targets, const u32 *__restrict__ tlen,
-                                                   const uint8_t *__restrict__ mask, u64 excl, u64 *__restrict__ top) {
+                                                   const uint8_t *__restrict__ mask, u64 excl, u64 *__restrict__ top, PartRef pr) {
     __shared__ u64 wtot[16];
     const u32 c = blockIdx.x * 1024u + threadIdx.x;
     u64 total;
-    (void)block_incl_scan_u64(c < n_targets ? hist_bins_of<MODE>(&ctg[c], c, tlen, mask, excl) : 0, wtot, total);
+    (void)block_incl_scan_u64(c < n_targets && pr.contig_in(c) ? hist_bins_of<MODE>(&ctg[c], c, tlen, mask, excl) : 0, wtot, total);
     if (threadIdx.x == 0) top[blockIdx.x] = total;
 }
 template <int MODE>
 __global__ __launch_bounds__(1024) void k_hist_off(DevContig *ctg, u32 n_targets, const u32 *__restrict__ tlen, const uint8_t *__restrict__ mask,
-                                                   u64 excl, const u64 *__restrict__ top, DevGlobal *g) {
+                                                   u64 excl, const u64 *__restrict__ top, DevGlobal *g, PartRef pr) {
     __shared__ u64 wtot[16];
     u64 mine = 0, base;
     for (u32 b = threadIdx.x; b < blockIdx.x; b += 1024u) mine += top[b];
     (void)block_incl_scan_u64(mine, wtot, base);
+    if (pr.part == PART_B) base += pr.cut->arena_a;
     const u32 c = blockIdx.x * 1024u + threadIdx.x;
-    const u64 v = c < n_targets ? hist_bins_of<MODE>(&ctg[c], c, tlen, mask, excl) : 0;
+    const bool in = c < n_targets && pr.contig_in(c);
+    const u64 v = in ? hist_bins_of<MODE>(&ctg[c], c, tlen, mask, excl) : 0;
     u64 total;
     const u64 inc = block_incl_scan_u64(v, wtot, total);
-    if (c < n_targets) {
+    if (in) {
         if (MODE == 0) ctg[c].hist_off = base + inc - v;
         else { ctg[c].chist_off = base + inc - v; ctg[c].hist_len = (u32)v; }
     }
     if (blockIdx.x == gridDim.x - 1 && threadIdx.x == 0) {
-        if (MODE == 0) g->hist_cap_total = base + total; else g->chist_total = base + total;
-    }
-}
-
-__global__ void k_zero_u32(u32 *__restrict__ p, const u64 *__restrict__ n_ptr) {
-    const u64 n = *n_ptr;
-    for (u64 i = (u64)blockIdx.x * blockDim.x + threadIdx.x; i < n; i += (u64)gridDim.x * blockDim.x) p[i] = 0u;
+        if (MODE == 0) { if (pr.part == PART_A) pr.cut->arena_a = base + total; else g->hist_cap_total = base + total; }
+        else g->chist_total = base + total;
+    }
+}
+
+__global__ void k_zero_u32(u32 *__restrict__ p, const u64 *__restrict__ lo_ptr, const u64 *__restrict__ n_ptr) {
+    const u64 lo = lo_ptr != nullptr ? *lo_ptr : 0ull, n = *n_ptr;
+    for (u64 i = lo + (u64)blockIdx.x * blockDim.x + threadIdx.x; i < n; i += (u64)gridDim.x * blockDim.x) p[i] = 0u;
 }
 
 __global__ __launch_bounds__(256) void k_hist_compact(const DevContig *__restrict__ ctg, u32 n_targets,
@@ -1188,6 +1235,8 @@
     int32_t *depth_out;
     const u64 *depth_off;
     u32 tile_base;
+    u32 part;
+    const SplitCut *cut;
 };
 
 
@@ -1510,11 +1559,14 @@
         r0 = i0 < d.y ? a.runs[i0] : make_uint2(0u, 0u);
         r1 = i1 < d.y ? a.runs[i1] : make_uint2(0u, 0u);
     };
+    u32 tile_base = a.tile_base;
+    if (a.part == PART_A) n_tiles = min(n_tiles, a.cut->tile_cut);
+    else if (a.part == PART_B) { tile_base = min(n_tiles, a.cut->tile_cut); n_tiles -= tile_base; }
     const u32 n_chunks = (n_tiles + chunk_tiles - 1) / chunk_tiles;
     if (wave_id >= n_chunks) return;
     u32 ch = wave_id;
     u32 t = ch * chunk_tiles, t_end = min(t + chunk_tiles, n_tiles);
-    uint4 ds = a.desc[2 * (size_t)(a.tile_base + t)], dC1 = a.desc[2 * (size_t)(a.tile_base + t) + 1];
+    uint4 ds = a.desc[2 * (size_t)(tile_base + t)], dC1 = a.desc[2 * (size_t)(tile_base + t) + 1];
     uint2 rw0, rw1;
     load_runs(ds, rw0, rw1);
     for (;;) {
@@ -1528,7 +1580,7 @@
         }
         const bool have_next = tn != 0xffffffffu;
         uint4 nds = make_uint4(0u, 0u, 0u, 0u), ndC1 = make_uint4(0u, 0u, 0u, 0u);
-        if (have_next) { nds = a.desc[2 * (size_t)(a.tile_base + tn)]; ndC1 = a.desc[2 * (size_t)(a.tile_base + tn) + 1]; }
+        if (have_next) { nds = a.desc[2 * (size_t)(tile_base + tn)]; ndC1 = a.desc[2 * (size_t)(tile_base + tn) + 1]; }
 
         const u32 c = dC1.x, lo = dC1.y, L = ds.z, cxo = dC1.z, cxn = dC1.w;
         const bool live = (ds.x < ds.y || cxn != 0u) && !(ds.w & TILE_F_SLOW);
diff --git a/coverm_amd/csrc/prep_lean.hip.h b/coverm_amd/csrc/prep_lean.hip.h
--- a/coverm_amd/csrc/prep_lean.hip.h
+++ b/coverm_amd/csrc/prep_lean.hip.h
@@ -185,7 +185,7 @@
         if (qm != 0) {
             const int ql = __ffsll((long long)qm) - 1;
             u32 b = 0;
-            if (lane == ql) b = atomicAdd(&g->n_cx, (u32)__popcll(qm));
+            if (lane == ql) b = atomicAdd(cd.n_cx, (u32)__popcll(qm));
             b = __builtin_amdgcn_readlane(b, ql);
             const u32 rank = __builtin_amdgcn_mbcnt_hi((u32)(qm >> 32), __builtin_amdgcn_mbcnt_lo((u32)qm, 0u));
             if (is_bucket && b + rank < cd.cx_list_cap) cd.cx_list[b + rank] = i;
@@ -288,7 +288,7 @@
     const int lane = lane_id();
     const u32 w = (u32)__builtin_amdgcn_readfirstlane((int)(threadIdx.x >> 6));
     const u32 wave_recs = h.steps * 64u;
-    const u32 base = (blockIdx.x * 4u + w) * wave_recs;
+    const u32 base = ((blockIdx.x + cold->blk0) * 4u + w) * wave_recs;
     bool flushed_early = false;
     LeanAcc acc; acc.reset();
     int cur = -1;
@@ -448,18 +448,19 @@
     }
     if (lane == 0) { blk_cnt[0][w] = g_prim; blk_cnt[1][w] = g_cons; wmask[w] = left_mask; }
     __syncthreads();
+    const u32 blk = ((base >> 6) / h.steps) >> 2;
     if (w == 0u) {
         const u32 m0 = wmask[0], m1 = wmask[1], m2 = wmask[2], m3 = wmask[3];
         const u32 c0 = (u32)__popc(m0), c1 = c0 + (u32)__popc(m1), c2 = c1 + (u32)__popc(m2), total = c2 + (u32)__popc(m3);
         if (total) {
             u32 at = 0;
-            if (lane == 0) at = atomicAdd(&cold->g->n_gen, total);
+            if (lane == 0) at = atomicAdd(cold->n_gen, total);
             at = (u32)__builtin_amdgcn_readfirstlane((int)at);
             for (u32 e = (u32)lane; e < total; e += 64u) {
                 const u32 k = e < c0 ? 0u : e < c1 ? 1u : e < c2 ? 2u : 3u;
                 u32 m = k == 0u ? m0 : k == 1u ? m1 : k == 2u ? m2 : m3;
                 for (u32 r = e - (k == 0u ? 0u : k == 1u ? c0 : k == 2u ? c1 : c2); r != 0u; r--) m &= m - 1u;
-                cold->gen_list[at + e] = (blockIdx.x * 4u + k) * wave_recs + (u32)__builtin_ctz(m) * 64u;
+                cold->gen_list[at + e] = (blk * 4u + k) * wave_recs + (u32)__builtin_ctz(m) * 64u;
             }
         }
     }
@@ -482,14 +483,14 @@
                     o.first = min(o.first, q.first); o.last = max(o.last, q.last); o.nm += q.nm; o.indel += q.indel;
                 }
             }
-            cold->part[blockIdx.x] = o;
+            cold->part[blk] = o;
         }
     }
     if (!uniform_wg) lean_flush(cold->ctg, cur, acc);
     if (threadIdx.x == 0) {
         const u32 p = blk_cnt[0][0] + blk_cnt[0][1] + blk_cnt[0][2] + blk_cnt[0][3];
         const u32 c = blk_cnt[1][0] + blk_cnt[1][1] + blk_cnt[1][2] + blk_cnt[1][3];
-        const u32 slot = (blockIdx.x % COUNTER_SLOTS) * 8u;
+        const u32 slot = (blk % COUNTER_SLOTS) * 8u;
         DevGlobal *g = cold->g;
         if (p) atomicAdd(&g->prim_slots[slot], (u64)p);
         if (c) atomicAdd(&g->cons_slots[slot], (u64)c);
@@ -502,7 +503,7 @@
 }
 template <bool WANT_IDENTITY, bool FILTER, bool MASKED>
 __global__ __launch_bounds__(256) void k_prep_generic(const PrepArgs *__restrict__ pa, u32 all_steps) {
-    const u32 n = all_steps ? all_steps : pa->cold.g->n_gen;
+    const u32 n = all_steps ? all_steps : *pa->cold.n_gen;
     const u32 *__restrict__ list = pa->cold.gen_list;
     for (u32 j = blockIdx.x * 4u + (threadIdx.x >> 6); j < n; j += gridDim.x * 4u) {
         const u32 i0 = all_steps ? j * 64u : (u32)__builtin_amdgcn_readfirstlane((int)list[j]);
diff --git a/coverm_amd/engine.py b/coverm_amd/engine.py
--- a/coverm_amd/engine.py
+++ b/coverm_amd/engine.py
@@ -273,6 +273,11 @@
         self._check(self._lib.cov_last_paths(self._h, C.byref(v)))
         return dict(listed_steps=int(v[0]), generic_only=bool(v[1]), slow_tiles=int(v[2]), bucket_records=int(v[3]))
 
+    def last_split(self):
+        v = (C.c_uint32 * 4)()
+        self._check(self._lib.cov_last_split(self._h, C.byref(v)))
+        return dict(split=bool(v[0]), fell_back=bool(v[1]), cut_record=int(v[2]), cut_contig=int(v[3]))
+
     def algorithmic_bytes(self):
         b = C.c_uint64(0)
         self._check(self._lib.cov_algorithmic_bytes(self._h, C.byref(b)))
diff --git a/coverm_amd/native.py b/coverm_amd/native.py
--- a/coverm_amd/native.py
+++ b/coverm_amd/native.py
@@ -54,7 +54,7 @@
 
 EXPORTS = ["cov_abi_version", "cov_create", "cov_destroy", "cov_last_error", "cov_set_targets",
            "cov_set_target_mask", "cov_push_batch", "cov_push_batch_device", "cov_finish", "cov_fetch_hist",
-           "cov_copy_depth", "cov_reset", "cov_kernel_ms", "cov_algorithmic_bytes", "cov_last_paths",
+           "cov_copy_depth", "cov_reset", "cov_kernel_ms", "cov_algorithmic_bytes", "cov_last_paths", "cov_last_split",
            "cov_set_genomes", "cov_finish_genomes", "cov_fetch_genome_estimates", "cov_fetch_genome_stats",
            "cov_set_genome_runs", "cov_genome_entry_count", "cov_fetch_genome_entries",
            "cov_sam_begin", "cov_sam_window_bytes", "cov_sam_slot_wait", "cov_sam_feed", "cov_sam_end"]
@@ -105,6 +105,7 @@
     L.cov_kernel_ms.argtypes = [C.c_void_p, C.c_int, C.POINTER(C.c_double), C.POINTER(C.c_uint32)]
     L.cov_algorithmic_bytes.argtypes = [C.c_void_p, C.POINTER(C.c_uint64)]
     L.cov_last_paths.argtypes = [C.c_void_p, C.POINTER(C.c_uint32 * 4)]
+    L.cov_last_split.argtypes = [C.c_void_p, C.POINTER(C.c_uint32 * 4)]
     L.cov_set_estimators.argtypes = [C.c_void_p, C.c_void_p, C.c_uint32]
     L.cov_fetch_estimates.argtypes = [C.c_void_p, C.c_void_p]
     L.cov_set_genomes.argtypes = [C.c_void_p, C.c_void_p, C.c_uint32]
diff --git a/include/covermhip.h b/include/covermhip.h
--- a/include/covermhip.h
+++ b/include/covermhip.h
@@ -168,6 +168,8 @@
 cov_status cov_kernel_ms(const cov_session *s, cov_kernel_id k, double *ms_total, uint32_t *launches);
 typedef struct { uint32_t listed_steps, generic_only, slow_tiles, bucket_records; } cov_path_counts;
 cov_status cov_last_paths(const cov_session *s, cov_path_counts *out);
+typedef struct { uint32_t split, fell_back, cut_record, cut_contig; } cov_split_info;
+cov_status cov_last_split(const cov_session *s, cov_split_info *out);
 cov_status cov_algorithmic_bytes(const cov_session *s, uint64_t *bytes);
 
 typedef struct {
```

Result: slower. 49.05 billion (-2.7%).
